# RNG65536/CUDA-volpath

Hardware: AMD Instinct MI355X
Metric: Msamples/sec (WxHxspp) + achieved HBM GB/s, Julia 256^3 @ 800x600 (higher is better)
Workload: dtype f32; 1 GPU; julia256_800x600_global_majorant; image=800x600, estimator=global_majorant, bound_brick=1, rng=philox2x32-7, parallelism=pixel-tiles x1

## Files before the change

cuda-volpath_amd/csrc/vp_context.cpp:

```cpp
#include "vp_state.h"

namespace vph __attribute__((visibility("hidden")))
{
State                      g_default;
static thread_local State* t_current = nullptr;
State& cur() { return t_current ? *t_current : g_default; }

int fail(int code, const char* fmt, ...)
{
    char    buf[512];
    va_list ap;
    va_start(ap, fmt);
    vsnprintf(buf, sizeof buf, fmt, ap);
    va_end(ap);
    G.err = buf;
    return code;
}
[[noreturn]] void die(const char* what)
{
    fprintf(stderr, "volpath_hip: %s: %s\n", what, G.err.c_str());
    exit(EXIT_FAILURE);
}
int ensure_device()
{
// ... 13 lines not shown
    G.num_cu = prop.multiProcessorCount;
    HIPCHK(hipStreamCreateWithFlags(&G.own_stream, hipStreamNonBlocking));
    if (!G.stream) G.stream = G.own_stream;
    HIPCHK(hipMalloc((void**)&G.d_queue, 2 * kTargets * kQueueWords * sizeof(unsigned)));
    HIPCHK(hipMalloc((void**)&G.d_counters, kCounterWords * sizeof(unsigned long long)));
    HIPCHK(hipMemset(G.d_counters, 0, kCounterWords * sizeof(unsigned long long)));
    HIPCHK(hipMalloc((void**)&G.d_cancel, 3 * sizeof(unsigned)));
    HIPCHK(hipMemset(G.d_cancel, 0, 3 * sizeof(unsigned)));
    G.S.sun_cos = 94.0f / sqrtf(94.0f * 94.0f + 0.45f * 0.45f);
    G.S.cam_z   = (float)(-1.0f / tan((double)54.43f * 0.00872664626));
    auto knob = [](const char* name, long lo, long hi, long& out) {
        const char* e = getenv(name);
        if (!e || !*e) return false;
        char* end = nullptr;
        long  v   = strtol(e, &end, 10);
        if (*end || v < lo || v > hi)
        {
            fprintf(stderr, "volpath_hip: ignoring %s=%s (allowed %ld..%ld)\n", name, e, lo, hi);
            return false;
        }
        out = v;
        return true;
    };
    long v;
    if (knob("VP_WAIT_LANES", 1, 64, v)) { G.wait_lanes = (unsigned)v; G.wait_lanes_set = true; }
    if (knob("VP_WAIT_ITERS", VP_STEPS_PER_PASS, 1 << 20, v)) G.wait_iters = (unsigned)v;
    if (knob("VP_SETUP_LANES", 1, 64, v)) G.setup_lanes = (unsigned)v;
    if (knob("VP_END_LANES", 1, 64, v)) G.end_lanes = (unsigned)v;
    if (knob("VP_LIGHT_WAIT_ITERS", VP_STEPS_PER_PASS, 1 << 20, v)) G.light_wait_iters = (unsigned)v;
    if (knob("VP_STAGE_MB", 1, 256 << 10, v)) G.max_stage_bytes = (size_t)v << 20;
    if (knob("VP_BLOCKS_PER_CU", 1, 8, v)) G.blocks_per_cu = (unsigned)v;
    {
        long kmax = 0;
        while ((VP_CHUNK >> (kmax + 1)) >= 1) kmax++;
        if (knob("VP_CHUNK_FRAMES_LOG2", 0, kmax, v)) G.chunk_fshift = (unsigned)v;
    }
    if (knob("VP_NO_LDS_BOUNDS", 0, 1, v)) G.use_lds_bounds = v == 0;
    if (knob("VP_NO_LDS_HELPER", 0, 1, v)) G.lds_helper = v == 0;
    if (knob("VP_NO_LDS_COMPACT", 0, 1, v)) G.use_lds_compact = v == 0;
    if (knob("VP_LDS_COMPACT_CHROMATIC", 0, 1, v)) G.lds_compact_chromatic = v != 0;
    if (knob("VP_LDS_PAIRS", 0, 1, v)) G.lds_pairs = v != 0;
    if (knob("VP_CELL_BRICKS", 0, 1, v)) G.cell_bricks = (int)v;
    if (knob("VP_NO_CRAWL_TABLE", 0, 1, v)) G.use_crawl_table = v == 0;
    if (knob("VP_NO_EMPTY_TABLE", 0, 1, v)) G.use_empty_table = v == 0;
    if (knob("VP_NO_SUN_CLIP", 0, 1, v)) G.use_sun_clip = v == 0;
    if (knob("VP_DENSE_PERCENT", 0, 101, v)) G.dense_fraction = (float)v / 100.0f;
    if (knob("VP_NO_OPACITY_LDS", 0, 1, v)) G.opacity_lds = v == 0;
    if (knob("VP_NO_OPACITY_CELLS", 0, 1, v)) G.use_opacity_cells = v == 0;
    if (knob("VP_NO_LIGHT_CONST", 0, 1, v)) G.use_light_const = v == 0;
    if (knob("VP_NO_CONST_ROWS", 0, 1, v)) G.use_const_rows = v == 0;
    if (knob("VP_NO_APPROACH", 0, 1, v)) G.use_approach = v == 0;
    if (knob("VP_NO_APPROACH_LOCAL", 0, 1, v)) G.use_approach_local = v == 0;
    if (knob("VP_NO_APPROACH_TABLE", 0, 1, v)) G.use_approach_table = v == 0;
    if (knob("VP_APPROACH_FRAMES_LOG2", 0, 6, v)) G.approach_fshift_max = (unsigned)v;
    if (knob("VP_APPROACH_STEPS", 0, 1 << 30, v)) G.approach_steps = (unsigned)v;
    if (knob("VP_NO_LIGHT", 0, 1, v)) G.use_light = v == 0;
    if (knob("VP_NO_LIGHT_OVERLAP", 0, 1, v)) G.light_overlap = v == 0;
    if (knob("VP_NO_LIGHT_LOCAL", 0, 1, v)) G.use_light_local = v == 0;
    if (knob("VP_DEBUG_ONLY_CLASS", 0, 1, v)) G.debug_only_class = (int)v;
    if (knob("VP_GENERAL_BLOCKS_PER_CU", 1, 8, v)) G.general_blocks_per_cu = (unsigned)v;
    if (knob("VP_LIGHT_BLOCKS_PER_CU", 1, 8, v)) G.light_blocks_per_cu = (unsigned)v;
    if (knob("VP_THR_TABLE", 2, 1 << 20, v)) G.thr_entries = (unsigned)v;
    if (knob("VP_LOOKAHEAD", 0, 4096, v)) G.la_max = (int)v;
    if (knob("VP_LOOKAHEAD_OVERLAP_FROM", 1, 4096, v)) G.la_overlap_from = (int)v;
    if (knob("VP_LOOKAHEAD_RAMP_FROM", 2, 4096, v)) G.la_ramp_from = (int)v;
    if (knob("VP_LOOKAHEAD_FLOOR", 1, 4096, v)) G.la_floor = (int)v;
    if (knob("VP_LOOKAHEAD_DIV", 1, 16, v)) G.la_div = (int)v;
    if (knob("VP_LOOKAHEAD_NO_SPECULATION", 0, 1, v)) G.la_speculate = v == 0;
    if (knob("VP_NO_LA_CANCEL", 0, 1, v)) G.la_cancel = v == 0;
    if (knob("VP_NO_PIPELINE", 0, 1, v)) G.pipeline = v == 0;
    if (knob("VP_NO_EXIT", 0, 1, v)) G.use_exit = v == 0;
    if (knob("VP_EXIT_LOCAL", 0, 1, v)) { G.exit_local = v != 0; G.exit_local_auto = false; }
    if (knob("VP_EXIT_K", 1, VP_EXIT_TRIP, v)) G.exit_k = (unsigned)v;
    G.dev_ready = true;
    return VP_OK;
}


hipError_t create_internal_stream(hipStream_t* st)
{
    int lo = 0, hi = 0;
    if (hipDeviceGetStreamPriorityRange(&lo, &hi) != hipSuccess) { (void)hipGetLastError(); lo = hi = 0; }
    return hipStreamCreateWithPriority(st, hipStreamNonBlocking, lo);
}

int free_volume()
{
    G.epoch++;
    (void)la_quiesce();

    if (G.d_cells) HIPCHK(hipFree(G.d_cells));
    if (G.d_bounds) HIPCHK(hipFree(G.d_bounds));
    if (G.d_opacity) HIPCHK(hipFree(G.d_opacity));
    if (G.d_opacity_cells) { if (G.opacity_cells_on_host) HIPCHK(hipHostFree(G.h_opacity_cells)); else HIPCHK(hipFree(G.d_opacity_cells)); }
    G.d_opacity_cells = nullptr; G.h_opacity_cells = nullptr; G.S.opacity_cells = nullptr; G.opacity_cells_on_host = false;
    if (G.d_bound_codes) HIPCHK(hipFree(G.d_bound_codes));
    G.d_bound_codes = nullptr; G.bound_codes_ok = false;
    if (G.d_danger) HIPCHK(hipFree(G.d_danger));
    G.d_danger = nullptr;
    if (G.d_sunclip) HIPCHK(hipFree(G.d_sunclip));
    G.d_sunclip = nullptr; G.sunclip_key.clear();
    if (G.d_exit) HIPCHK(hipFree(G.d_exit));
    G.d_exit = nullptr;
    G.d_cells = G.d_bounds = nullptr;
    G.d_opacity   = nullptr;
    G.S.cells_u8  = nullptr;
// ... 337 lines not shown
        fail(VP_E_NODEVICE, "vp_ctx_create: device %d not visible (%d devices)", device, n);
        return nullptr;
    }
    vp_ctx* c = new vp_ctx();
    c->st.device = device;
    State* prev = t_current;
    t_current   = &c->st;
    int rc      = ensure_device();
    std::string why = c->st.err;
    t_current   = prev;
    if (rc)
    {
        delete c;
        fail(rc, "vp_ctx_create(%d): %s", device, why.c_str());
        return nullptr;
    }
    return c;
}
int vp_ctx_set_current(vp_ctx* ctx)
{
    t_current = ctx ? &ctx->st : nullptr;
    if (G.dev_ready) HIPCHK(hipSetDevice(G.device));
    return VP_OK;
}
vp_ctx* vp_ctx_get_current(void) { return t_current ? reinterpret_cast<vp_ctx*>(t_current) : nullptr; }
int vp_ctx_device(void) { return G.device; }
int vp_ctx_destroy(vp_ctx* ctx)
{
    if (!ctx) return VP_OK;
    State* prev = t_current;
    t_current   = &ctx->st;
    State& D    = ctx->st;
    int rc = VP_OK;
    if (D.dev_ready)
    {
        (void)hipSetDevice(D.device);
        (void)hipStreamSynchronize(D.stream);
        (void)la_quiesce();
        rc = free_volume();
        free_envmap();
        for (auto& sl : D.la)
        {
            if (sl.done) (void)hipEventDestroy(sl.done);
            if (sl.stream) (void)hipStreamDestroy(sl.stream);
        }
        for (auto& ev : D.events) { (void)hipEventDestroy(ev.first); (void)hipEventDestroy(ev.second); }
        for (auto& ev : D.class_events) { (void)hipEventDestroy(ev.a); (void)hipEventDestroy(ev.b); }
        for (auto e : D.event_pool) (void)hipEventDestroy(e);
        (void)pipe_quiesce();
        for (hipStream_t st : D.pipe_stream) if (st) (void)hipStreamDestroy(st);
        for (hipEvent_t e : {D.pipe_done[0], D.pipe_done[1], D.pipe_free[0], D.pipe_free[1], D.pipe_gate[0], D.pipe_gate[1], D.pipe_fence_ev, D.last_end,
                             D.class_last_end[0], D.class_last_end[1], D.class_last_end[2]})
            if (e) (void)hipEventDestroy(e);
        D.d_crawl.release(); D.d_seg.release(); D.d_sub_cls.release(); D.d_tiles.release(); D.d_act.release(); D.d_act_scratch.release();
        for (void* q : {(void*)D.d_thr, (void*)D.d_sunclip, (void*)D.d_bound_codes, (void*)D.d_light_flag, (void*)D.d_tile_rows, (void*)D.d_tile_scratch})
            if (q) (void)hipFree(q);
        for (RenderTarget& t : D.target)
        {
            if (t.aux_stream) { (void)hipStreamSynchronize(t.aux_stream); (void)hipStreamDestroy(t.aux_stream); }
            t.stage.release();
            t.handover.release();
            for (hipEvent_t e : t.aux_ev) if (e) (void)hipEventDestroy(e);
        }
        if (D.d_queue) (void)hipFree(D.d_queue);
        if (D.d_counters) (void)hipFree(D.d_counters);
        if (D.ctrl_stream) (void)hipStreamDestroy(D.ctrl_stream);
        if (D.d_cancel) (void)hipFree(D.d_cancel);
        if (D.own_stream) (void)hipStreamDestroy(D.own_stream);
    }
    t_current = (prev == &ctx->st) ? nullptr : prev;
    delete ctx;
    if (G.dev_ready) (void)hipSetDevice(G.device);
    return rc;
}
int vp_accumulate(vp_float4* dst, const vp_float4* src, size_t n)
{
    int rc = ensure_device();
    if (rc) return rc;
    if (!dst || !src) return fail(VP_E_ARG, "vp_accumulate: null pointer");
    if (n) launch_accumulate((float4*)dst, (const float4*)src, n, G.stream);
    HIPCHK(hipGetLastError());
    return VP_OK;
}
int vp_tile_owner(unsigned tx, unsigned ty, int world)
{
    if (world < 1) return -1;
    return (int)((tx + vp::tile_row_shift(ty, (unsigned)world)) % (unsigned)world);
}
int vp_set_stream(void* s)
{
    int rc = ensure_device();
    if (rc) return rc;
    HIPCHK(hipStreamSynchronize(G.stream));
    if (la_quiesce()) return VP_E_NODEVICE;
    G.stream = s ? (hipStream_t)s : G.own_stream;
    return VP_OK;
}
void* vp_get_stream(void)
{
    if (ensure_device()) return nullptr;
    return (void*)G.stream;
}
int vp_synchronize(void)
{
    int rc = ensure_device();
    if (rc) return rc;
    HIPCHK(hipStreamSynchronize(G.stream));
// ... 12 lines not shown
    if (mode != VP_RNG_SAMPLERH && mode != VP_RNG_PHILOX && mode != VP_RNG_PHILOX7) return fail(VP_E_ARG, "unknown rng %d", mode);
    G.rng = mode; G.key0 = k0; G.key1 = k1;
    return VP_OK;
}
int vp_set_exit_flights(int mode)
{
    if (mode < 0 || mode > 2) return fail(VP_E_ARG, "exit flights: 0 off, 1 global-majorant estimator (default), 2 every estimator that has them");
    int rc = ensure_device();
    if (rc || (rc = pipe_quiesce())) return rc;
    G.use_exit = mode != 0; G.exit_local = mode == 2; G.exit_local_auto = false;
    if (G.use_exit && G.have_volume && !G.d_exit && G.d_danger)
    {
        if (la_quiesce()) return VP_E_NODEVICE;
        const size_t n = (size_t)G.S.nx * G.S.ny * G.S.nz;
        if (hipMalloc((void**)&G.d_exit, 3 * n) == hipSuccess)
        {
            launch_exit_table(G.d_danger, G.d_exit, G.S.nx, G.S.ny, G.S.nz, G.stream);
            HIPCHK(hipGetLastError());
        }
        else { (void)hipGetLastError(); G.d_exit = nullptr; }
    }
    return VP_OK;
}
int vp_set_tracking(int mode)
{
    if (int rc = pipe_quiesce()) return rc;
    if (mode != VP_TRACK_SPECTRAL && mode != VP_TRACK_SCALAR && mode != VP_TRACK_MULTI_CHANNEL)
        return fail(VP_E_ARG, "unknown tracking mode %d", mode);
    G.trk = mode;
    return VP_OK;
}
int vp_set_lookahead(int max_frames)
{
    if (max_frames < 0 || max_frames > 4096) return fail(VP_E_ARG, "look-ahead of %d frames out of range [0,4096]", max_frames);
    if (la_quiesce()) return VP_E_NODEVICE;
    G.la_max = max_frames; G.la_prev_n = 0;
    return VP_OK;
}
int vp_set_arithmetic(int mode)
{
    if (mode != VP_ARITH_EXACT && mode != VP_ARITH_FAST) return fail(VP_E_ARG, "unknown arithmetic mode %d", mode);
    if (mode == G.arith) return VP_OK;
    if (la_quiesce()) return VP_E_NODEVICE;
    G.arith = mode;
    return VP_OK;
}
int vp_set_subpixel(int s)
{
    const int shift = subpixel_shift_of(s);
    if (shift < 0) return fail(VP_E_ARG, "sub-pixel factor %d: 1, 2, 4 or 8", s);
    if (shift == G.sub_shift) return VP_OK;
    if (la_quiesce()) return VP_E_NODEVICE;
    G.sub_shift = shift;
    G.crawl_key.clear(); G.tiles_key.clear(); G.seg_key.clear();
    return VP_OK;
}
int vp_get_subpixel(void) { return 1 << G.sub_shift; }
int vp_subpixel_offset(unsigned x, unsigned y, int frame, int s, int* i, int* j)
{
    const int shift = subpixel_shift_of(s);
    if (shift < 0) return fail(VP_E_ARG, "sub-pixel factor %d: 1, 2, 4 or 8", s);
    if (x > 0xffffu || y > 0xffffu || frame < 0) return fail(VP_E_ARG, "vp_subpixel_offset: pixel (%u, %u) or frame %d out of range", x, y, frame);
    unsigned oi = 0, oj = 0;
    vp::subpixel_offset(x, y, (unsigned)frame, (unsigned)shift, oi, oj);
    if (i) *i = (int)oi;
    if (j) *j = (int)oj;
    return VP_OK;
}
int vp_set_envmap_sampling(int mode)
{
    if (int rc = pipe_quiesce()) return rc;
    if (mode != VP_ENV_PASSIVE && mode != VP_ENV_MIS) return fail(VP_E_ARG, "unknown environment sampling mode %d", mode);
    int rc = ensure_device();
    if (rc) return rc;
    G.env_mis = mode == VP_ENV_MIS;
    if (G.env_mis) return build_env_tables();
    return VP_OK;
}
int vp_get_env_tables(float* cdf_y, float* cdf_x, float* pdfnorm_alt)
{
    int rc = ensure_device();
    if (rc) return rc;
    if (!G.env_tables) return fail(VP_E_STATE, "no environment tables: vp_set_envmap_sampling(VP_ENV_MIS) and init_envmap first");
    HIPCHK(hipStreamSynchronize(G.stream));
    if (cdf_y) HIPCHK(hipMemcpy(cdf_y, G.d_env_cdf_y, (size_t)G.env_h * sizeof(float), hipMemcpyDeviceToHost));
    if (cdf_x) HIPCHK(hipMemcpy(cdf_x, G.d_env_cdf_x, (size_t)G.env_w * G.env_h * sizeof(float), hipMemcpyDeviceToHost));
    if (pdfnorm_alt) *pdfnorm_alt = G.S.env_pdfnorm_alt;
    return VP_OK;
}
int vp_init_volume(const void* h_volume, vp_extent ext, int format, const vp_float3* bmin, const vp_float3* bmax)
{
    if (!h_volume) return fail(VP_E_ARG, "vp_init_volume: null volume");
    if (format != VP_VOL_U8 && format != VP_VOL_F32 && format != VP_VOL_F16) return fail(VP_E_ARG, "vp_init_volume: unknown volume format %d", format);
    if (ext.width == 0 || ext.height == 0 || ext.depth == 0) return fail(VP_E_ARG, "empty volume extent");
    return do_init_volume(h_volume, ext, format, bmin, bmax);
}
int vp_get_volume_info(vp_volume_info* out)
{
    if (!out) return fail(VP_E_ARG, "vp_get_volume_info: null result");
    if (!G.have_volume) return fail(VP_E_STATE, "no volume");
    out->format = G.vol_format;
    out->nx = G.S.nx; out->ny = G.S.ny; out->nz = G.S.nz;
    out->cell_bytes  = G.quant ? 8 : (G.half() ? 16 : 32);
    out->cells_bytes = (uint64_t)G.cells_bytes;
    return VP_OK;
}
int vp_set_bound_brick(int brick)
// ... 162 lines not shown
    unsigned *dn = (unsigned*)D.get(c * 32), *dr = (unsigned*)D.get(c * 32);
    if (!dor || !db || !dn || !dr) return fail(VP_E_NOMEM, "vp_test_sun_start: no device memory");
    HIPCHK(hipMemcpy(dor, origin_xyz, c * 12, hipMemcpyHostToDevice));
    HIPCHK(hipMemcpy(db, box, 24, hipMemcpyHostToDevice));
    if (G.arith == VP_ARITH_FAST) launch_test_sun_start_fast(n, dor, sun_dir, db, dn, dr, G.stream);
    else launch_test_sun_start(n, dor, sun_dir, db, dn, dr, G.stream);
    HIPCHK(hipStreamSynchronize(G.stream));
    HIPCHK(hipMemcpy(out_new, dn, c * 32, hipMemcpyDeviceToHost));
    HIPCHK(hipMemcpy(out_ref, dr, c * 32, hipMemcpyDeviceToHost));
    return VP_OK;
}
int vp_test_hg(const float* g, const float* r0, const float* r1, const float* normal_xyz, const float* cos_query, float* dir_xyz, float* eval, int n)
{
    int rc = ensure_device();
    if (rc) return rc;
    if (n <= 0) return VP_OK;
    DevArrays D;
    const size_t b = (size_t)n * 4;
    float *dg = (float*)D.get(b), *d0 = (float*)D.get(b), *d1 = (float*)D.get(b), *dn = (float*)D.get(3 * b), *dc = (float*)D.get(b);
    float *dd = (float*)D.get(3 * b), *de = (float*)D.get(b);
    if (!dg || !d0 || !d1 || !dn || !dc || !dd || !de) return fail(VP_E_NOMEM, "vp_test_hg: no device memory");
    HIPCHK(hipMemcpy(dg, g, b, hipMemcpyHostToDevice));
    HIPCHK(hipMemcpy(d0, r0, b, hipMemcpyHostToDevice));
    HIPCHK(hipMemcpy(d1, r1, b, hipMemcpyHostToDevice));
    HIPCHK(hipMemcpy(dn, normal_xyz, 3 * b, hipMemcpyHostToDevice));
    HIPCHK(hipMemcpy(dc, cos_query, b, hipMemcpyHostToDevice));
    if (G.arith == VP_ARITH_FAST) launch_test_hg_fast(dg, d0, d1, dn, dc, dd, de, n, G.stream);
    else launch_test_hg(dg, d0, d1, dn, dc, dd, de, n, G.stream);
    HIPCHK(hipStreamSynchronize(G.stream));
    HIPCHK(hipMemcpy(dir_xyz, dd, 3 * b, hipMemcpyDeviceToHost));
    HIPCHK(hipMemcpy(eval, de, b, hipMemcpyDeviceToHost));
    return VP_OK;
}
int vp_test_intersect_box(const float* origin_xyz, const float* dir_xyz, int* hit, float* tnear, float* tfar, int n)
{
    if (!G.have_volume) return fail(VP_E_STATE, "no volume (the box comes from init_cuda)");
    int rc = ensure_device();
    if (rc) return rc;
    if (n <= 0) return VP_OK;
    DevArrays D;
    const size_t b = (size_t)n * 4;
    float *dor = (float*)D.get(3 * b), *ddi = (float*)D.get(3 * b), *dtn = (float*)D.get(b), *dtf = (float*)D.get(b);
    int*   dh  = (int*)D.get(b);
    if (!dor || !ddi || !dtn || !dtf || !dh) return fail(VP_E_NOMEM, "vp_test_intersect_box: no device memory");
    HIPCHK(hipMemcpy(dor, origin_xyz, 3 * b, hipMemcpyHostToDevice));
    HIPCHK(hipMemcpy(ddi, dir_xyz, 3 * b, hipMemcpyHostToDevice));
    launch_test_box(G.S, dor, ddi, dh, dtn, dtf, n, G.stream);
    HIPCHK(hipStreamSynchronize(G.stream));
    HIPCHK(hipMemcpy(hit, dh, b, hipMemcpyDeviceToHost));
    HIPCHK(hipMemcpy(tnear, dtn, b, hipMemcpyDeviceToHost));
    HIPCHK(hipMemcpy(tfar, dtf, b, hipMemcpyDeviceToHost));
    return VP_OK;
}
int vp_test_eval_envmap(const float* dir_xyz, float* rgb, int n)
{
    if (!G.have_env) return fail(VP_E_STATE, "no environment map");
    int rc = ensure_device();
    if (rc) return rc;
    if (n <= 0) return VP_OK;
    DevArrays D;
    const size_t b = (size_t)n * 12;
    float *dd = (float*)D.get(b), *dq = (float*)D.get(b);
    if (!dd || !dq) return fail(VP_E_NOMEM, "vp_test_eval_envmap: no device memory");
    HIPCHK(hipMemcpy(dd, dir_xyz, b, hipMemcpyHostToDevice));
    launch_test_env(G.S, dd, dq, n, G.stream);
    HIPCHK(hipStreamSynchronize(G.stream));
    HIPCHK(hipMemcpy(rgb, dq, b, hipMemcpyDeviceToHost));
    return VP_OK;
}

int vp_julia_voxelize(int n, unsigned char* host_out)
{
    int rc = ensure_device();
    if (rc) return rc;
    if (n < 1 || n > 1024 || !host_out) return fail(VP_E_ARG, "bad julia grid size %d", n);
    size_t total = (size_t)n * n * n;
    unsigned char* d = nullptr;
    HIPCHK(hipMalloc((void**)&d, total));
    launch_julia(d, n, G.stream);
    HIPCHK(hipGetLastError());
    HIPCHK(hipStreamSynchronize(G.stream));
    HIPCHK(hipMemcpy(host_out, d, total, hipMemcpyDeviceToHost));
    HIPCHK(hipFree(d));
    return VP_OK;
}

int vp_cloud_voxelize(int n, uint32_t seed, float* host_out)
{
    int rc = ensure_device();
    if (rc) return rc;
    if (n < 1 || n > 1024 || !host_out) return fail(VP_E_ARG, "bad cloud grid size %d", n);
    size_t total = (size_t)n * n * n;
    float* d = nullptr;
    HIPCHK(hipMalloc((void**)&d, total * sizeof(float)));
    launch_cloud(d, n, seed, G.stream);
    hipError_t e = hipGetLastError();
    if (e == hipSuccess) e = hipStreamSynchronize(G.stream);
    if (e == hipSuccess) e = hipMemcpy(host_out, d, total * sizeof(float), hipMemcpyDeviceToHost);
    (void)hipFree(d);
    if (e != hipSuccess) return fail(VP_E_NODEVICE, "vp_cloud_voxelize -> %s", hipGetErrorString(e));
    return VP_OK;
}

void* vp_malloc(size_t bytes)
{
    if (ensure_device()) return nullptr;
// ... 38 lines not shown
```

cuda-volpath_amd/csrc/vp_integrator.h:

```cpp
enum : int
{
    ST_DONE    = 0,
    ST_SETUP   = 1,
    ST_TRACK   = 2,
    ST_SHADOW  = 3,
    EV_SCATTER = 4,
    EV_NEE     = 5,
    EV_BG      = 6,
    EV_WRITE   = 7,
    EV_MIS     = 8,
    EV_HG      = 9
};

#ifndef VP_PAD_STEP
#define VP_PAD_STEP 0
#endif
#ifndef VP_PAD_FETCH
#define VP_PAD_FETCH 0
#endif
#ifndef VP_PAD_EOF
#define VP_PAD_EOF 0
#endif
#ifndef VP_PAD_SETUP
#define VP_PAD_SETUP 0
// ... 90 lines not shown
    {
        const float reduction   = (1.0f - s) + s * (1.0f - P.g);
        const float cur_density = reduction * P.density;
        const float d_max       = fmaxf(0.0001f, (float)b * VP_U8_SCALE);
        sigma_t_prime           = max_sig * cur_density * d_max;
    }
    else
    {
        const float cur_density = (1.0f - s) * P.density + s * P.density * (1.0f - P.g);
        sigma_t_prime           = max_sig * cur_density;
    }
    const float inv_sigma_t = rcp_(sigma_t_prime);
    if (!(null_collision_in_empty_space(1.0f, sigma_t_prime, inv_sigma_t) == 1.0f)) atomicAnd(flag, 0u);
}

#ifndef VP_LOCAL_MIN_WAVES
#define VP_LOCAL_MIN_WAVES 6
#endif
constexpr int render_min_waves(int est, bool count, int ldsb, bool ach, bool mis, int trk, bool light, bool cancel)
{
    if (VP_MIN_WAVES > 1) return VP_MIN_WAVES;
    if (light) return count ? 5 : (est != EST_GLOBAL ? VP_LIGHT_LOCAL_MIN_WAVES : VP_LIGHT_MIN_WAVES);
    if (mis || ldsb == 1) return 1;
    if (count) return 4;
    if (est == EST_GLOBAL && trk == 0) return VP_GLOBAL_MIN_WAVES;
    if (trk) return 4;
    return (ach && !cancel) ? VP_LOCAL_MIN_WAVES : 5;
}
#define VP_RENDER_K_HAS_LAYERS 1
template <int EST, class RNG, bool QUANT, bool COUNT, int LDSB, bool ACH, bool MIS, int TRK, bool LIGHT = false, bool CANCEL = false, bool HALF = false, bool LYR = false>
__global__ __launch_bounds__(LDSB == 1 ? VP_BLOCK_LDS : VP_BLOCK, render_min_waves(EST, COUNT, LDSB, ACH, MIS, TRK, LIGHT, CANCEL))
void render_k(SceneDev S, LaunchDev L)
{
    __shared__ unsigned short lds_bounds[LDSB == 1 ? VP_LDS_BOUND_ENTRIES : 1];
    __shared__ unsigned lds_codes[LDSB == 2 ? VP_LDS_BOUND_ENTRIES / 16 : 1];
    if (LDSB == 2)
    {
        const uint4* src = reinterpret_cast<const uint4*>(L.bound_codes);
        uint4*       dst = reinterpret_cast<uint4*>(lds_codes);
        const int    n16 = (S.bnx * S.bny * S.bnz + 63) / 64;
        for (int w = threadIdx.x; w < n16; w += VP_BLOCK) dst[w] = src[w];
        __syncthreads();
    }
    if (LDSB == 1)
    {
        const uint4* src = reinterpret_cast<const uint4*>(S.bounds_u8);
        uint4*       dst = reinterpret_cast<uint4*>(lds_bounds);
        const int    n16 = (S.bnx * S.bny * S.bnz * 2 + 15) / 16;
        for (int w = threadIdx.x; w < n16; w += VP_BLOCK_LDS) dst[w] = src[w];
        __syncthreads();
    }
    constexpr unsigned KARG_L_   = ((sizeof(SceneDev) + alignof(LaunchDev) - 1) / alignof(LaunchDev)) * alignof(LaunchDev);
    constexpr unsigned KARG_WDS_ = (KARG_L_ + sizeof(LaunchDev) + 3) / 4;
    constexpr bool LOCAL = EST != EST_GLOBAL;
    constexpr bool TAB   = TRK == 0 && LDSB != 1 && !LIGHT && !MIS;
#ifdef VP_EXP_BOX_PARALLEL
    constexpr bool SUNROW = false;
#else
    constexpr bool SUNROW = TAB && EST != EST_BOUNDED;
#endif
    __shared__ __attribute__((aligned(16))) unsigned kargs_lds_[KARG_WDS_ + (SUNROW ? SR_WORDS : 0)];
    {
        const unsigned* src = (const unsigned*)__builtin_amdgcn_kernarg_segment_ptr();
        for (unsigned w = threadIdx.x; w < KARG_WDS_; w += (LDSB == 1 ? VP_BLOCK_LDS : VP_BLOCK)) kargs_lds_[w] = src[w];
    }
    __shared__ __attribute__((aligned(16))) float coll_tab_[TAB ? VP_COLL_ROWS : 1][CR_WORDS];
    if (TAB && threadIdx.x < VP_COLL_ROWS)
        coll_row_fill(coll_tab_[threadIdx.x], (int)threadIdx.x, L.P.g, L.P.density, max3(f3{L.P.sigma_t[0], L.P.sigma_t[1], L.P.sigma_t[2]}), LOCAL);
    if (SUNROW && threadIdx.x == VP_COLL_ROWS)
        sun_row_fill(reinterpret_cast<float*>(kargs_lds_ + KARG_WDS_), f3{S.sun_dir[0], S.sun_dir[1], S.sun_dir[2]});
    __syncthreads();
    auto coll_row = [&](int n) __attribute__((always_inline)) -> const float* {
        return TAB ? coll_tab_[n < 0 ? 0 : (n > VP_COLL_ROWS - 1 ? VP_COLL_ROWS - 1 : n)] : nullptr;
    };
    constexpr bool EARLY = RNG::kShadowSubstream && !MIS && !LIGHT;
    constexpr bool APPR = EST == EST_GLOBAL && TRK == 0 && !LIGHT && !MIS;
    constexpr bool APPR_L = EST == EST_DECOMP && TRK == 0 && !LIGHT && !MIS;
    constexpr bool EXITC = TRK == 0 && !MIS && !LIGHT && EST != EST_BOUNDED && (QUANT || EST == EST_GLOBAL);
    constexpr bool PARK = !MIS;
    constexpr bool DEFER = EARLY && TRK == 0;
    constexpr bool LAYERS = LYR;
    static_assert(!LYR || (TRK == 0 && !MIS && !COUNT && !CANCEL), "layers instances: spectral tracking, passive environment, no counters, no look-ahead");
    const ParamDev& P = L.P;
    const f3    sig_t     = f3{P.sigma_t[0], P.sigma_t[1], P.sigma_t[2]};
    const f3    sig_s     = sig_t * f3{P.albedo[0], P.albedo[1], P.albedo[2]};
    const float max_sig   = max3(sig_t);
    const float min_sig   = min3(sig_t);
    const float density   = P.density;

    int      st = ST_DONE;
    bool     exhausted = false;
    constexpr bool COLD = LDSB != 1 && !LIGHT;
    constexpr int  CS_  = COLD ? VP_BLOCK : 1;
    constexpr int NCOLD = 14 + (DEFER ? (ACH ? 1 : 3) : 0);
    static_assert(!COLD || (LOCAL ? VP_LOCAL_MIN_WAVES : VP_GLOBAL_MIN_WAVES) * (NCOLD * VP_BLOCK * 4 + KARG_WDS_ * 4 + VP_COLL_ROWS * CR_WORDS * 4 + (SUNROW ? SR_WORDS * 4 : 0) + (LDSB == 2 ? VP_LDS_BOUND_ENTRIES / 4 : 0)) <= VP_LDS_BYTES_PER_CU,
                  "cold per-path state: more workgroups per CU than the LDS holds -- lower VP_*_MIN_WAVES for this ARCH");
    __shared__ float cold_[COLD ? NCOLD : 1][CS_];
    float* const cold_p = &cold_[0][COLD ? threadIdx.x : 0];
    ColdF3<COLD, CS_>       rad(cold_p), pd(cold_p + 3 * CS_);
    ColdVal<float, COLD>    ph(cold_p + 6 * CS_), phase_g(cold_p + 7 * CS_);
    ColdVal<unsigned, COLD> item(cold_p + 8 * CS_);
    ColdVal<unsigned, COLD> px(cold_p + 9 * CS_), py(cold_p + 10 * CS_);
    ColdVal<int, COLD>      frame(cold_p + 11 * CS_);
    ColdVal<int, COLD>      nsc(cold_p + 12 * CS_);
    ColdVal<unsigned, COLD> rng_saved(cold_p + 13 * CS_);
    constexpr unsigned LIGHT_NONE = 0xffffffffu;
    ColdVal<float, COLD>    lw_x(cold_p + 6 * CS_), lw_y(cold_p + (DEFER && !ACH ? 14 : 6) * CS_), lw_z(cold_p + (DEFER && !ACH ? 15 : 6) * CS_);
    ColdVal<unsigned, COLD> light_bits(cold_p + (DEFER ? NCOLD - 1 : 6) * CS_);
    if (COLD) { rad = f3{0.0f, 0.0f, 0.0f}; pd = f3{0.0f, 0.0f, 0.0f}; ph = 0.0f; phase_g = 0.0f; item = 0u; px = 0u; py = 0u; frame = 0; nsc = 0; rng_saved = 0u; }
    if (DEFER) { lw_x = 0.0f; if (!ACH) { lw_y = 0.0f; lw_z = 0.0f; } light_bits = LIGHT_NONE; }
    RNG      rng;
    f3       ro = {}, rd = {};
    f3       inv_rd = {};
    f3       thr = {};
    int      seg = 0;
    float    dist = 0, t_end = 0;
    float    t_far = 0, distc = 0, inv_sigma = 0, inv_sigma_t = 0, sigma_t_prime = 0, sigma_c = 0;
    float    cur_density = 0, d_max = 0;
    f3       nee_a = {};
    int      terms = 0;
    f3       nee_c = {}, nee_t = {}, seg_o = {};
    int      nee_stage = 0;
    float    sh_inv_sigma = 0, sh_density = 0;
    float    sig_base = density;
    int      chan = 0;
    float    t_empty = 0.0f;
    float    t_clip = 1e30f;
    bool     ex_clear = false;
    unsigned long long c_load = 0, c_xtest = 0, c_xout = 0, c_xok = 0;
    unsigned zrun = 0;

    unsigned long long c_den = 0, c_bnd = 0, c_opa = 0, c_env = 0, c_sca = 0, c_smp = 0;
    unsigned long long d_iter = 0, d_act = 0, d_outer = 0, d_shadow = 0;
    constexpr bool PROF = COUNT && VP_PROFILE_BLOCKS;
    unsigned long long t_slow = 0, t_fast = 0, t_mark = PROF ? __builtin_amdgcn_s_memtime() : 0ull;
    enum { B_SETUP, B_HALF, B_LOOK, B_EXIT, B_SCATTER, B_NEE, B_HG, B_BG, B_WRITE, B_REFILL, B_GSETUP, B_FETCH, B_ZERO, B_ZERO_SH, B_EXITT, B_NBLK };
    unsigned long long bw[B_NBLK] = {}, bl[B_NBLK] = {};
    unsigned long long hist[3][8] = {};
    unsigned long long ctrl_w = 0, ctrl_l = 0;
    auto tally = [&](int b, bool on) __attribute__((always_inline)) {
        if (PROF)
        {
            unsigned long long m = __ballot(on);
            if (m)
            {
                bw[b] += 1; bl[b] += (unsigned)__popcll(m);
                const int h = b == B_SCATTER ? 0 : b == B_EXIT ? 1 : b == B_SETUP ? 2 : -1;
                if (h >= 0) hist[h][((unsigned)__popcll(m) - 1u) >> 3] += 1;
            }
        }
    };

    const unsigned lane = threadIdx.x & 63u;
    unsigned chunk_s = 0, chunk_n = 0;
    unsigned chunk_q = 0, chunk_f0 = 0;
    bool     queue_empty = false;
    unsigned q_cur   = __builtin_amdgcn_s_getreg((4 - 1) << 11 | 20) & (VP_NQUEUES - 1);
    unsigned q_tried = 0;
    unsigned end_skipped = 0;
    unsigned visits = 0;

    for (;;)
    {
        if (PROF && lane == 0) d_outer++;
        {
#ifdef VP_EXP_FLAT_KARGS
        const char* kargs_ = (const char*)__builtin_amdgcn_kernarg_segment_ptr();
        asm volatile("" : "+s"(kargs_));
#else
        unsigned ko_ = 0;
        asm volatile("" : "+v"(ko_));
        const char* kargs_ = reinterpret_cast<const char*>(kargs_lds_) + ko_;
#endif
        const SceneDev&  S = *reinterpret_cast<const SceneDev*>(kargs_);
        const LaunchDev& L = *reinterpret_cast<const LaunchDev*>(kargs_ + KARG_L_);
        const ParamDev&  P = L.P;
        const f3 sun_dir   = f3{S.sun_dir[0], S.sun_dir[1], S.sun_dir[2]};
        const f3 sun_power = f3{S.sun_power[0], S.sun_power[1], S.sun_power[2]};
        auto start_shadow = [&](f3 end, float inv_s, float den, unsigned stage) __attribute__((always_inline)) {
            f3    sd;
            float len, tn, tf;
            bool  hitv;
            if (SUNROW && stage == 0u)
            {
#ifdef VP_EXP_FLAT_KARGS
                const float* const srow = reinterpret_cast<const float*>(kargs_lds_ + KARG_WDS_);
#else
                const float* const srow = reinterpret_cast<const float*>(kargs_ + KARG_WDS_ * 4u);
#endif
                hitv = sun_start(srow, ro, S.bmin, S.bmax, sd, len, tn, tf);
            }
            else
            {
                const f3    dv = end - ro;
                const float d2 = dot(dv, dv);
                len = sqrt_(d2);
#ifdef VP_ARITH_FAST
                sd = dv * rsqrt_(d2);
#else
                sd = dv * rcp_(len);
#endif
                hitv = intersect_box(ro, sd, S, tn, tf);
            }
            if (!hitv)
            {
                nee_a = f3{1.0f, 1.0f, 1.0f};
                st    = EV_NEE;
            }
            else
            {
                if (tn < 0.0f) tn = 0.0f;
                t_end       = fminf(tf, len);
                dist        = tn;
                terms       = 0;
                rd          = sd;
                inv_sigma   = inv_s;
                cur_density = den;
                st          = ST_SHADOW;
                rng_saved = rng.enter_shadow(2u * (unsigned)(int)nsc + stage);
                if (COUNT) t_clip = 1e30f;
                if (RNG::kShadowSubstream && stage == 0u && L.sun_clip)
                {
                    f3    pl = to_local(S, ro);
                    int   ci, cj, ck;
                    float w_;
                    axis_linear(pl.x, S.nx, ci, w_);
                    axis_linear(pl.y, S.ny, cj, w_);
                    axis_linear(pl.z, S.nz, ck, w_);
                    const unsigned n = L.sun_clip[(size_t)((unsigned)ci + __umul24((unsigned)S.nx, (unsigned)cj + __umul24((unsigned)S.ny, (unsigned)ck)))];
                    if (n != 0xffffu)
                    {
                        const float tc = (float)n * L.clip_ds;
                        if (COUNT && !L.count_clips) t_clip = tc;
                        else t_end = fminf(t_end, tc);
                    }
                }
            }
        };
        auto segment_medium = [&]() __attribute__((always_inline)) {
            if (LOCAL && TAB) cur_density = coll_row(nsc - 5)[CR_DENS];
            else if (LOCAL)
// ... 210 lines not shown
                const f3 pl = to_local(S, st == ST_TRACK ? ro + rd * dist : ro);
                int   ci, cj, ck;
                float w_;
                axis_linear(pl.x, S.nx, ci, w_);
                axis_linear(pl.y, S.ny, cj, w_);
                axis_linear(pl.z, S.nz, ck, w_);
                const float ex = rd.x * (S.linv[0] * (float)S.nx), ey = rd.y * (S.linv[1] * (float)S.ny), ez = rd.z * (S.linv[2] * (float)S.nz);
                const float ax = __builtin_fabsf(ex), ay = __builtin_fabsf(ey), az = __builtin_fabsf(ez);
                const unsigned A   = (ax >= ay && ax >= az) ? 0u : (ay >= az ? 1u : 2u);
                const unsigned cls = A == 0u ? ((ex > 0.0f ? 1u : 0u) | (ey > 0.0f ? 2u : 0u) | (ez > 0.0f ? 4u : 0u))
                                   : A == 1u ? ((ey > 0.0f ? 1u : 0u) | (ex > 0.0f ? 2u : 0u) | (ez > 0.0f ? 4u : 0u))
                                             : ((ez > 0.0f ? 1u : 0u) | (ex > 0.0f ? 2u : 0u) | (ey > 0.0f ? 4u : 0u));
                const size_t   ncell = (size_t)S.nx * (size_t)S.ny * (size_t)S.nz;
                const unsigned bits  = L.exit_oct[(size_t)A * ncell + (size_t)((unsigned)ci + __umul24((unsigned)S.nx, (unsigned)cj + __umul24((unsigned)S.ny, (unsigned)ck)))];
                bool clear = (bits >> cls) & 1u;
                bool unit = true;
                if (clear)
                {
                    const f3 t3 = ACH ? f3{thr.x, thr.x, thr.x} : thr;
                    if (LOCAL)
                    {
                        for (unsigned q = 0; q < L.exit_nbytes; q++)
                        {
                            const float dm  = fmaxf(0.0001f, (float)((L.exit_bytes >> (8u * q)) & 0xffu) * VP_U8_SCALE);
                            const float stp = max_sig * cur_density * dm;
                            unit = unit && null_collision_is_identity(t3, stp, rcp_(stp));
                        }
                    }
                    else
                        unit = null_collision_is_identity(t3, sigma_t_prime, inv_sigma_t);
                }
                if (COUNT && clear && unit) c_xok++;
                if (clear && unit && !(COUNT && !L.count_clips)) st = EV_BG;
                else
                {
                    if (COUNT && clear && unit) ex_clear = true;
                    terms = (clear && unit) ? -(1 << 30) : (unit ? L.exit_start : L.exit_start - 4 * VP_EXIT_TRIP);
                }
            }
        }
        {
            const unsigned long long wantm = __ballot(st == EV_BG || st == EV_WRITE || (st == ST_DONE && !exhausted) || (EST == EST_GLOBAL && st == ST_SETUP));
            const bool fast_any = __ballot(st == ST_TRACK || st == ST_SHADOW || (LOCAL && st == ST_SETUP)) != 0ull;
            end_skipped++;
            if (wantm == 0ull || (!LIGHT && fast_any && (unsigned)__popcll(wantm) < L.end_lanes && end_skipped < 4u)) goto ends_done;
            end_skipped = 0u;
        }
#pragma unroll 1
        for (int rep = 0; rep < 4; rep++)
        {
            vp_pad<VP_PAD_END>();
            bool fresh = false;
            bool trans = false;
            tally(B_BG, st == EV_BG);
            if (st == EV_BG)
            {
                if (!MIS || nsc == 0)
                {
                    if (LAYERS) trans = nsc == 0;
                    f3 bg;
                    if (LAYERS && trans) bg = f3{1.0f, 1.0f, 1.0f};
                    else if (nsc == 0 && dot(rd, sun_dir) > S.sun_cos) bg = f3{S.sun_orig[0], S.sun_orig[1], S.sun_orig[2]};
                    else { bg = eval_envmap(S, rd); if (COUNT) c_env++; }
                    if (LIGHT && !LOCAL)
                    {
                        const unsigned n = (unsigned)seg, last = L.thr_n - 1u;
                        float t = L.thr_table[n < last ? n : last];
                        for (unsigned k = last; k < n; k++) t = null_collision_in_empty_space(t, sigma_t_prime, inv_sigma_t);
                        thr = f3{t, t, t};
                    }
                    rad = rad + bg * (ACH ? f3{thr.x, thr.x, thr.x} : thr);
                }
                st = EV_WRITE;
            }
            tally(B_WRITE, st == EV_WRITE);
            if (st == EV_WRITE)
            {
                f3     r    = rad * ((LAYERS && trans) ? 1.0f : P.brightness);
#ifdef VP_ARITH_FAST
                r = f3{r.x < __builtin_inff() ? r.x : 0.0f, r.y < __builtin_inff() ? r.y : 0.0f, r.z < __builtin_inff() ? r.z : 0.0f};
#endif
                float  heat = (EST == EST_DECOMP) ? (float)nsc : (float)((double)(EST == EST_BOUNDED ? seg : nsc) * 0.001);
                if (LAYERS && !LIGHT && trans) heat = -heat;
                float4 v    = make_float4(fmaxf(r.x, 0.0f), fmaxf(r.y, 0.0f), fmaxf(r.z, 0.0f), heat);
                if (TRK == 2)
                    v = make_float4(chan == 0 ? v.x * 3.0f : 0.0f, chan == 1 ? v.y * 3.0f : 0.0f, chan == 2 ? v.z * 3.0f : 0.0f, heat);
                if (L.stage) L.stage[item] = v;
                else
                {
                    size_t idx = (size_t)px + (size_t)py * P.width;
                    float4 a   = L.out[idx];
                    L.out[idx] = make_float4(a.x + v.x, a.y + v.y, a.z + v.z, a.w + v.w);
                }
                st = ST_DONE;
            }
            {
                bool               need = (st == ST_DONE) && !exhausted;
                unsigned long long m    = __ballot(need);
                tally(B_REFILL, need);
                if (m)
                {
                    while (chunk_s >= chunk_n && !queue_empty)
                    {
                        const unsigned q0 = L.q_start[q_cur], len = L.q_start[q_cur + 1] - q0;
                        static_assert((VP_CHUNK & (VP_CHUNK - 1)) == 0 && VP_CHUNK >= 64, "VP_CHUNK: a power of two, at least a wave");
                        const unsigned sh = L.chunk_fshift, ppc = (unsigned)VP_CHUNK >> sh, fblocks = (unsigned)L.nframes >> sh;
                        const unsigned cpf = (len + ppc - 1u) / ppc;
                        unsigned c = 0xffffffffu;
                        if (len)
                        {
                            if (lane == 0 && !(L.cancel && __hip_atomic_load(L.cancel, __ATOMIC_RELAXED, __HIP_MEMORY_SCOPE_AGENT) >= L.batch_id)) c = atomicAdd(L.queue + q_cur * VP_QUEUE_STRIDE, 1u);
                            c = __builtin_amdgcn_readfirstlane(c);
                        }
                        if (c < cpf * fblocks)
                        {
                            const unsigned pos = c / fblocks, fb = c - pos * fblocks, off = pos * ppc;
                            chunk_q  = q0 + off;
                            chunk_f0 = fb << sh;
                            chunk_n  = (len - off < ppc ? len - off : ppc) << sh;
                            chunk_s  = 0;
                        }
                        else
                        {
                            q_cur = (q_cur + 1) & (VP_NQUEUES - 1);
                            if (++q_tried >= VP_NQUEUES) queue_empty = true;
                        }
                    }
                    unsigned cnt   = (unsigned)__popcll(m);
                    unsigned avail = chunk_n - chunk_s;
                    unsigned take  = cnt < avail ? cnt : avail;
                    unsigned rank  = lane_rank(m);
                    if (need)
                    {
                        if (rank >= take) { if (queue_empty) exhausted = true;  }
                        else
                        {
                            const unsigned sn  = chunk_s + rank, sh = L.chunk_fshift;
                            const unsigned rem = chunk_q + (sn >> sh);
                            const unsigned fl  = chunk_f0 + (sn & ((1u << sh) - 1u));
                            item = fl * L.stage_stride + L.slot_base + rem;
                            unsigned pix = L.pixels[rem];
                            px    = pix & 0xffffu;
                            py    = pix >> 16;
                            frame = L.frame0 + (int)fl;
                            if (px < P.width && py < P.height)
                            {
                                auto table_index = [&]() -> size_t
                                {
                                    if (!COUNT && L.sub_shift)
                                    {
                                        unsigned si, sj;
                                        subpixel_offset(px, py, (unsigned)frame, L.sub_shift, si, sj);
                                        return (size_t)((px << L.sub_shift) + si) + (size_t)((py << L.sub_shift) + sj) * (P.width << L.sub_shift);
                                    }
                                    return (size_t)px + (size_t)py * P.width;
                                };
                                if (!COUNT && L.sub_shift)
                                {
                                    unsigned si, sj;
                                    subpixel_offset(px, py, (unsigned)frame, L.sub_shift, si, sj);
                                    const unsigned fx = (px << L.sub_shift) + si, fy = (py << L.sub_shift) + sj;
                                    rng.init(fx, fy, (unsigned)frame, L.key0, L.key1);
                                    camera_ray(S, P.width << L.sub_shift, P.height << L.sub_shift, fx, fy, ro, rd);
                                }
                                else
                                {
                                    rng.init(px, py, (unsigned)frame, L.key0, L.key1);
                                    camera_ray(S, P.width, P.height, px, py, ro, rd);
                                }
                                if (TRK == 2)
                                {
                                    chan     = (int)fminf((1.0f - rng.next_a()) * 3.0f, 2.9999998f);
                                    sig_base = density * (chan == 0 ? P.sigma_t[0] : chan == 1 ? P.sigma_t[1] : P.sigma_t[2]);
                                }
                                if (LOCAL) inv_rd = f3{1.0f / rd.x, 1.0f / rd.y, 1.0f / rd.z};
                                thr = f3{1.0f, 1.0f, 1.0f};
                                rad = f3{0.0f, 0.0f, 0.0f};
                                nsc = 0;
                                seg = 0;
                                if (EXITC) terms = L.exit_start;
                                if (COUNT) ex_clear = false;
                                if (!LIGHT) t_empty = L.crawl ? L.crawl[2 * table_index() + 1].x : 0.0f;
                                if (LOCAL) dist = -1.0f;
                                if (APPR && L.approach)
                                {
                                    const float4 a = L.stage[item];
                                    dist  = a.x;
                                    rng.load(f2u(a.y), f2u(a.z));
                                    fresh = true;
                                    if (L.approach == 2u)
                                    {
                                        const unsigned n = f2u(a.w), last = L.thr_n - 1u;
                                        float t = L.thr_table[n < last ? n : last];
                                        if (n > last)
                                        {
                                            const float s0  = hyperion_s(0 - 5);
                                            const float stp = max_sig * ((1.0f - s0) * density + s0 * density * (1.0f - P.g));
                                            const float inv = rcp_(stp);
                                            for (unsigned k = last; k < n; k++) t = null_collision_in_empty_space(t, stp, inv);
                                        }
                                        thr = f3{t, t, t};
                                    }
                                }
                                if (LOCAL && L.crawl)
                                {
                                    float4   c = L.crawl[2 * table_index()];
                                    unsigned k = f2u(c.w);
                                    ro = f3{c.x, c.y, c.z};
                                    if (!(APPR_L && L.approach)) rng.skip(k >> 16);
                                    if (EST == EST_BOUNDED) seg = (int)(k & 0xffffu);
                                    if (COUNT) c_bnd += k & 0xffffu;
                                    if (APPR_L && L.approach)
                                    {
                                        const float4 a  = L.stage[item];
                                        const uint2  ax = L.approach_aux[item];
                                        const f3     ra = f3{a.x, a.y, a.z};
                                        t_empty = t_empty - dot(ra - ro, rd) - 1e-4f;
                                        ro      = ra;
                                        dist    = a.w;
                                        rng.load(ax.x, ax.y);
                                    }
                                }
                                st  = ST_SETUP;
                                segment_medium();
                                if (COUNT) c_smp++;
                            }
                        }
                    }
                    chunk_s += take;
                }
            }
            if (EST == EST_GLOBAL) tally(B_GSETUP, st == ST_SETUP);
            if (EST == EST_GLOBAL && st == ST_SETUP)
            {
                float t_near, tf;
                bool  hit = intersect_box(ro, rd, S, t_near, tf);
                if (!hit) st = EV_BG;
                else
                {
                    if (t_near < 0.0f) t_near = 0.0f;
                    t_far         = tf;
                    t_end         = tf;
                    dist          = (APPR && fresh) ? dist : t_near;
                    float s       = hyperion_s(nsc - 5);
                    if (!TAB) phase_g = (1.0f - s) * P.g;
                    if (TAB)
                    {
                        const float* const row = coll_row(nsc - 5);
                        cur_density   = row[CR_DENS];
                        sigma_t_prime = row[CR_STP];
                    }
                    else if (TRK)
                    {
                        sigma_t_prime = (1.0f - s) * sig_base + s * sig_base * (1.0f - P.g);
                        cur_density   = sigma_t_prime;
                    }
                    else
                    {
                        cur_density   = (1.0f - s) * density + s * density * (1.0f - P.g);
                        sigma_t_prime = max_sig * cur_density;
                    }
                    inv_sigma     = TAB ? coll_row(nsc - 5)[CR_INV] : rcp_(sigma_t_prime);
                    inv_sigma_t   = inv_sigma;
                    st            = ST_TRACK;
                }
            }
            if (__ballot((st == ST_DONE && !exhausted) || st == EV_BG || st == EV_WRITE) == 0ull) break;
        }
ends_done:
        if (CANCEL && L.cancel && (visits++ & 7u) == 0u)
        {
            unsigned w = 0;
            if (lane == 0) w = __hip_atomic_load(L.cancel, __ATOMIC_RELAXED, __HIP_MEMORY_SCOPE_AGENT);
            if ((unsigned)__builtin_amdgcn_readfirstlane((int)w) >= L.batch_id) { st = ST_DONE; exhausted = true; queue_empty = true; }
        }
        if (__ballot(st != ST_DONE || !exhausted) == 0ull) break;
        }
        if (PROF) { unsigned long long t = __builtin_amdgcn_s_memtime(); if (lane == 0) t_slow += t - t_mark; t_mark = t; }

        auto segment_setup = [&]() __attribute__((always_inline)) {
            if (LOCAL) tally(B_SETUP, st == ST_SETUP);
            if (LOCAL && st == ST_SETUP)
            {
                vp_pad<VP_PAD_SETUP>();
                float t_near, tf;
                bool  hit = intersect_box_inv(ro, inv_rd, S, t_near, tf);
                t_near    = fmaxf(t_near, 0.0f);
                t_far     = fminf(tf, 0.05f);
                float bx, by;
// ... 636 lines not shown
```

cuda-volpath_amd/csrc/vp_kernels.h:

```cpp
#pragma once
#include <hip/hip_runtime.h>

#include "vp_device.h"

#define VP_BLOCK 256
#ifndef VP_BLOCK_LDS
#define VP_BLOCK_LDS 512
#endif
#ifndef VP_MIN_WAVES
#define VP_MIN_WAVES 1
#endif
#define VP_LDS_BYTES_PER_CU (160 * 1024)
#define VP_LDS_BOUND_ENTRIES 32768
#ifndef VP_CHUNK
#define VP_CHUNK 128
#endif
#define VP_NQUEUES 8
#define VP_QUEUE_STRIDE 16
#ifndef VP_WAIT_LANES
#define VP_WAIT_LANES 28
#endif
#ifndef VP_WAIT_ITERS
#define VP_WAIT_ITERS 16
#endif
// ... 21 lines not shown
#ifndef VP_STEPS_PER_PASS
#define VP_STEPS_PER_PASS 4
#endif
#define VP_EXIT_TRIP 64

namespace vp
{
__host__ __device__ inline unsigned tile_row_shift(unsigned ty, unsigned world) { return ((ty * 0x9E3779B1u) >> 15) % world; }
constexpr int EST_GLOBAL = 0, EST_DECOMP = 1, EST_BOUNDED = 2;
constexpr int RNG_SAMPLERH = 0, RNG_PHILOX = 1, RNG_PHILOX7 = 2;

struct LaunchDev
{
    ParamDev P;
    int      frame0, nframes;
    unsigned nslots;
    unsigned total_items;
    const unsigned* pixels;
    unsigned stage_stride;
    unsigned slot_base;
    float4*  out;
    float4*  stage;
    const float4* crawl;
    unsigned* queue;
    unsigned chunk_fshift;
    unsigned q_start[VP_NQUEUES + 1];
    unsigned long long* counters;
    unsigned key0, key1;
    unsigned wait_lanes, wait_iters;
    unsigned end_lanes;
    unsigned setup_lanes;
    const unsigned short* sun_clip;
    float    clip_ds;
    unsigned count_clips;
    const float* thr_table;
    unsigned thr_n;
    uint2*   approach_aux;
    unsigned approach;
    unsigned approach_fshift;
    unsigned approach_steps;
    const unsigned char* exit_oct;
    int      exit_start;
    unsigned exit_nbytes;
    unsigned exit_bytes;
    unsigned* cancel;
    unsigned  batch_id;
    unsigned      const_from;
    const float4* stage_const;
    const unsigned* bound_codes;
    unsigned        bound_pal[2];
    const float4* seg_table;
    unsigned sub_shift;
    unsigned layers;
};

[[noreturn]] void kernel_not_built();
constexpr int CENSUS_RENDER = 0, CENSUS_LAYERS = 1, CENSUS_APPROACH = 2;
void census_record(int unit, int kind, unsigned index);
size_t census_size(int kind);
void census_read(int unit, int kind, unsigned* launches, unsigned char* built, size_t count, bool reset);
void census_built(int kind, unsigned char* built, size_t count);
void census_built_fast(int kind, unsigned char* built, size_t count);
void launch_render(const SceneDev& S, const LaunchDev& L, int est, int rng, bool quant, bool half, bool count, int lds_form, bool mis, int trk,
                   int blocks, hipStream_t st);
void launch_render_fast(const SceneDev& S, const LaunchDev& L, int est, int rng, bool quant, bool half, bool count, int lds_form, bool mis, int trk,
                        int blocks, hipStream_t st);
void launch_render_light(const SceneDev& S, const LaunchDev& L, int est, int rng, bool quant, bool count, int blocks, hipStream_t st);
void launch_miss_fill(const SceneDev& S, const LaunchDev& L, bool local_estimator, hipStream_t st);
void launch_approach(const SceneDev& S, const LaunchDev& L, int est, int rng, bool quant, hipStream_t st);
void launch_approach_fast(const SceneDev& S, const LaunchDev& L, int est, int rng, bool quant, hipStream_t st);
unsigned segment_table_records(void);
void launch_segment_table(const SceneDev& S, unsigned width, unsigned height, const float4* crawl, const unsigned* pixels, unsigned nslots, float4* seg,
                          hipStream_t st);
void launch_thr_table(const ParamDev& P, float* table, unsigned count, hipStream_t st);
void launch_bound_bytes(const unsigned char* bounds, size_t nbricks, unsigned* mask, hipStream_t st);
void launch_light_identity(const ParamDev& P, bool local, const unsigned* mask, unsigned* flag, hipStream_t st);
void launch_light_identity_fast(const ParamDev& P, bool local, const unsigned* mask, unsigned* flag, hipStream_t st);
inline unsigned pixel_list_blocks(unsigned ntiles) { return (unsigned)(((size_t)ntiles * 64 + 1023) / 1024); }
void launch_pixel_lists(unsigned width, unsigned height, unsigned rank, unsigned world, unsigned ntiles, const unsigned* d_row_start,
                        const float4* table, const unsigned char* cls, unsigned* d_block_counts, unsigned* d_totals, unsigned* d_out, hipStream_t st);
void launch_subpixel_classes(const float4* fine, unsigned width, unsigned height, unsigned shift, unsigned char* cls, hipStream_t st);
void launch_env_tables(const float4* env, int w, int h, float* lum, float* row_sum, float* cdf_x, float* cdf_y, float* pdfnorm_alt,
                       hipStream_t st);
void launch_crawl_table(const SceneDev& S, bool quant, unsigned width, unsigned height, bool control_draw, const unsigned char* danger, float4* table,
                        hipStream_t st);
void launch_danger(const SceneDev& S, bool quant, bool half, unsigned char* out, unsigned long long* marked, hipStream_t st);
float sun_clip_step(const SceneDev& S);
void launch_sun_clip(const SceneDev& S, const unsigned char* danger, float ds, unsigned short* out, hipStream_t st);
void launch_empty_table(const SceneDev& S, unsigned width, unsigned height, const unsigned char* danger, float4* table, hipStream_t st);
void launch_exit_table(const unsigned char* danger, unsigned char* planes, int nx, int ny, int nz, hipStream_t st);
void launch_reduce(const LaunchDev& L, hipStream_t st);
void launch_reduce_layers(const LaunchDev& L, float4* trans, unsigned light_from, unsigned light_to, hipStream_t st);
struct PixelStatsDev { double sum_y, sum_y2; unsigned n, flags; };
struct StatsDev
{
    PixelStatsDev* stats;
    unsigned adaptive;
    unsigned min_frames;
    double   tol, fl;
};
void launch_reduce_stats(const LaunchDev& L, const StatsDev& T, hipStream_t st);
inline unsigned compact_blocks(unsigned n) { return (n + 1023u) / 1024u; }
void launch_compact_active(const unsigned* src, const unsigned n[3], unsigned width, const PixelStatsDev* stats, unsigned* d_block_counts,
                           unsigned* d_totals, unsigned* d_out, hipStream_t st);
void launch_scale_by_count(float4* dst, const float4* src, const PixelStatsDev* stats, int size, float s, hipStream_t st);
void launch_stats_rel_error(float* dst, const PixelStatsDev* stats, int size, float floor_y, hipStream_t st);
size_t denoise_lds_bytes(int R, int F);
void launch_denoise(float4* dst, const float4* src, const PixelStatsDev* stats, const float4* guide, const PixelStatsDev* gstats, int W, int H, int R,
                    int F, float k2, int form, hipStream_t st);
void launch_pack_u8(const unsigned char* vol, uint2* cells, int nx, int ny, int nz, bool bricks, hipStream_t st);
void launch_pack_f32(const float* vol, float* cells, int nx, int ny, int nz, bool bricks, hipStream_t st);
void launch_pack_f16(const unsigned short* vol, uint4* cells, int nx, int ny, int nz, bool bricks, hipStream_t st);
void launch_opacity(const SceneDev& S, bool quant, bool half, bool lds, const float dir[3], float* out, hipStream_t st);
void launch_build_bounds(const void* d_vol, bool quant, bool half, void* d_out, void* d_tmp_a, void* d_tmp_b, int nx, int ny, int nz, int radius, int brick,
                         hipStream_t st);
void launch_julia(unsigned char* grid, int n, hipStream_t st);
void launch_cloud(float* grid, int n, unsigned seed, hipStream_t st);
void launch_scale(float4* dst, const float4* src, int size, float s, hipStream_t st);
void launch_composite(float4* dst, const float4* fg, const float4* trans, const float4* plate, float r, float g, float b, int size, float s, hipStream_t st);
void launch_gamma(float4* dst, const float4* src, int size, float s, float inv_gamma, hipStream_t st);
void launch_accumulate(float4* dst, const float4* src, size_t n, hipStream_t st);
void launch_test_hg(const float* g, const float* r0, const float* r1, const float* nrm, const float* cosq, float* dir, float* ev, int n, hipStream_t st);
void launch_test_box(const SceneDev& S, const float* o, const float* d, int* hit, float* tn, float* tf, int n, hipStream_t st);
void launch_test_env(const SceneDev& S, const float* d, float* out, int n, hipStream_t st);
void launch_test_math(int which, const float* in, float* out, int n, hipStream_t st);
void launch_test_roots(int which, unsigned lo, unsigned hi, unsigned long long* mismatches, unsigned* first_bad, hipStream_t st);
void launch_test_hg_fast(const float* g, const float* r0, const float* r1, const float* nrm, const float* cosq, float* dir, float* ev, int n, hipStream_t st);
void launch_test_math_fast(int which, const float* in, float* out, int n, hipStream_t st);
void launch_test_log_forms(int which, unsigned lo, unsigned hi, unsigned long long* mismatches, unsigned* first_bad, hipStream_t st);
void launch_test_log_forms_fast(int which, unsigned lo, unsigned hi, unsigned long long* mismatches, unsigned* first_bad, hipStream_t st);
void launch_test_approach_walk(int kind, int n, const float* par, const unsigned* scr, const unsigned* words, unsigned* out_new, unsigned* out_ref, hipStream_t st);
void launch_test_approach_walk_fast(int kind, int n, const float* par, const unsigned* scr, const unsigned* words, unsigned* out_new, unsigned* out_ref,
                                    hipStream_t st);
void launch_test_sun_start(int n, const float* origin, const float* sun_dir, const float* box, unsigned* out_new, unsigned* out_ref, hipStream_t st);
void launch_test_sun_start_fast(int n, const float* origin, const float* sun_dir, const float* box, unsigned* out_new, unsigned* out_ref, hipStream_t st);
void launch_test_rng(int mode, unsigned x, unsigned y, unsigned f, unsigned k0, unsigned k1, int n, float* out, hipStream_t st);
void launch_test_density(const SceneDev& S, bool quant, bool half, const float* pos, float* out, int n, hipStream_t st);
}
```

cuda-volpath_amd/csrc/vp_kernels.hip:

```cpp
#include <hip/hip_runtime.h>

#include <atomic>
#include <cmath>
#include <cstdint>
#include <cstdio>
#include <cstdlib>
#include <utility>

#include "vp_device.h"
#include "vp_kernels.h"

namespace vp
{
#include "vp_integrator.h"

__global__ void thr_table_k(ParamDev P, float* table, unsigned count)
{
    if (threadIdx.x || blockIdx.x) return;
    const float max_sig       = max3(f3{P.sigma_t[0], P.sigma_t[1], P.sigma_t[2]});
    const float s             = hyperion_s(0 - 5);
    const float cur_density   = (1.0f - s) * P.density + s * P.density * (1.0f - P.g);
    const float sigma_t_prime = max_sig * cur_density;
    const float inv_sigma_t   = 1.0f / sigma_t_prime;
    float t = 1.0f;
// ... 563 lines not shown
    const unsigned k = t / L.nslots, slot = t - k * L.nslots;
    const ParamDev& P = L.P;
    const unsigned pix = L.pixels[slot], px = pix & 0xffffu, py = pix >> 16;
    const unsigned h = wang_hash(((px << 16) | py) ^ 0x9E3779B9u);
    unsigned fl = (k - ((unsigned)L.frame0 + h)) & (n2 - 1u);
    if (fl >= (unsigned)L.nframes) return;
    unsigned i, j;
    subpixel_offset(px, py, (unsigned)L.frame0 + fl, m, i, j);
    f3 ro, rd;
    camera_ray(S, P.width << m, P.height << m, (px << m) + i, (py << m) + j, ro, rd);
    bool env_lookup = false;
    const float4 v = unscattered_sample(S, P, rd, env_lookup, L.layers);
    if (L.stage)
        for (; fl < (unsigned)L.nframes; fl += n2) L.stage[(size_t)fl * L.stage_stride + L.slot_base + slot] = v;
    else
    {
        size_t idx = (size_t)px + (size_t)py * P.width;
        float4 a   = L.out[idx];
        L.out[idx] = make_float4(a.x + v.x, a.y + v.y, a.z + v.z, a.w + v.w);
    }
}

__global__ __launch_bounds__(256) void approach_segments_k(SceneDev S, unsigned width, unsigned height, const float4* crawl, const unsigned* pixels,
                                                           unsigned nslots, float4* seg)
{
    const unsigned slot = blockIdx.x * blockDim.x + threadIdx.x;
    if (slot >= nslots) return;
    float4* out = seg + (size_t)slot * (2 * VP_SEG_CAP);
    const unsigned pix = pixels[slot], px = pix & 0xffffu, py = pix >> 16;
    if (px >= width || py >= height) { out[0] = make_float4(0.0f, 0.0f, u2f(0x100u), 0.0f); out[VP_SEG_CAP] = make_float4(0.0f, 0.0f, 0.0f, 0.0f); return; }
    f3 ro, rd;
    camera_ray(S, width, height, px, py, ro, rd);
    const f3     inv_rd = f3{1.0f / rd.x, 1.0f / rd.y, 1.0f / rd.z};
    const size_t idx    = (size_t)px + (size_t)py * width;
    const float4 c      = crawl[2 * idx];
    float        t_empty = crawl[2 * idx + 1].x;
    ro                  = f3{c.x, c.y, c.z};
    for (unsigned n = 0; n < VP_SEG_CAP; n++)
    {
        float t_near, tf;
        const bool hit = intersect_box_inv(ro, inv_rd, S, t_near, tf);
        t_near         = fmaxf(t_near, 0.0f);
        const float t_far = fminf(tf, 0.05f);
        const f3  pl = to_local(S, ro + rd * t_near);
        const int bi = axis_point(pl.x, S.nx) >> S.brick_shift, bj = axis_point(pl.y, S.ny) >> S.brick_shift, bk = axis_point(pl.z, S.nz) >> S.brick_shift;
        const unsigned v = reinterpret_cast<const unsigned short*>(S.bounds_u8)[(size_t)((unsigned)bi + (unsigned)S.bnx * ((unsigned)bj + (unsigned)S.bny * (unsigned)bk))];
        const bool stop = !hit || (v >> 8) != 0u || n == VP_SEG_CAP - 1u;
        out[n]              = make_float4(t_near, t_far, u2f((v & 0xffu) | (stop ? 0x100u : 0u)), t_empty);
        out[VP_SEG_CAP + n] = make_float4(ro.x, ro.y, ro.z, 0.0f);
        if (stop) break;
        ro      = ro + rd * t_far;
        t_empty -= t_far;
    }
}

__device__ __forceinline__ size_t pack_index(int nx, int ny, int i, int j, int k, int bricks)
{
    if (!bricks) return (size_t)i + (size_t)nx * ((size_t)j + (size_t)ny * k);
    const size_t nbx = ((size_t)nx + 3) >> 2, nby = ((size_t)ny + 3) >> 2;
    return ((((size_t)i >> 2) + nbx * (((size_t)j >> 2) + nby * ((size_t)k >> 2))) << 6) | (size_t)(((k & 3) << 4) | ((j & 3) << 2) | (i & 3));
}
__global__ void pack_cells_u8_k(const unsigned char* vol, uint2* cells, int nx, int ny, int nz, int bricks)
{
    size_t n   = (size_t)nx * ny * nz;
    size_t idx = (size_t)blockIdx.x * blockDim.x + threadIdx.x;
    if (idx >= n) return;
    int i = (int)(idx % nx), j = (int)((idx / nx) % ny), k = (int)(idx / ((size_t)nx * ny));
    int i1 = i + 1 < nx ? i + 1 : nx - 1, j1 = j + 1 < ny ? j + 1 : ny - 1, k1 = k + 1 < nz ? k + 1 : nz - 1;
    auto at = [&](int a, int b, int c) -> unsigned { return vol[(size_t)a + (size_t)nx * ((size_t)b + (size_t)ny * c)]; };
    uint2 c;
    c.x = at(i, j, k) | (at(i1, j, k) << 8) | (at(i, j1, k) << 16) | (at(i1, j1, k) << 24);
    c.y = at(i, j, k1) | (at(i1, j, k1) << 8) | (at(i, j1, k1) << 16) | (at(i1, j1, k1) << 24);
    cells[pack_index(nx, ny, i, j, k, bricks)] = c;
}
__global__ void pack_cells_f32_k(const float* vol, float* cells, int nx, int ny, int nz, int bricks)
{
    size_t n   = (size_t)nx * ny * nz;
    size_t idx = (size_t)blockIdx.x * blockDim.x + threadIdx.x;
    if (idx >= n) return;
    int i = (int)(idx % nx), j = (int)((idx / nx) % ny), k = (int)(idx / ((size_t)nx * ny));
    int i1 = i + 1 < nx ? i + 1 : nx - 1, j1 = j + 1 < ny ? j + 1 : ny - 1, k1 = k + 1 < nz ? k + 1 : nz - 1;
    auto at = [&](int a, int b, int c) -> float { return vol[(size_t)a + (size_t)nx * ((size_t)b + (size_t)ny * c)]; };
    float4* q = reinterpret_cast<float4*>(cells) + pack_index(nx, ny, i, j, k, bricks) * 2;
    q[0] = make_float4(at(i, j, k), at(i1, j, k), at(i, j1, k), at(i1, j1, k));
    q[1] = make_float4(at(i, j, k1), at(i1, j, k1), at(i, j1, k1), at(i1, j1, k1));
}
__global__ void pack_f16_k(const unsigned short* vol, uint4* cells, int nx, int ny, int nz, int bricks)
{
    size_t n   = (size_t)nx * ny * nz;
    size_t idx = (size_t)blockIdx.x * blockDim.x + threadIdx.x;
    if (idx >= n) return;
    int i = (int)(idx % nx), j = (int)((idx / nx) % ny), k = (int)(idx / ((size_t)nx * ny));
    int i1 = i + 1 < nx ? i + 1 : nx - 1, j1 = j + 1 < ny ? j + 1 : ny - 1, k1 = k + 1 < nz ? k + 1 : nz - 1;
    auto at = [&](int a, int b, int c) -> unsigned { return vol[(size_t)a + (size_t)nx * ((size_t)b + (size_t)ny * c)]; };
    cells[pack_index(nx, ny, i, j, k, bricks)] = make_uint4(at(i, j, k) | (at(i1, j, k) << 16), at(i, j1, k) | (at(i1, j1, k) << 16),
                                                            at(i, j, k1) | (at(i1, j, k1) << 16), at(i, j1, k1) | (at(i1, j1, k1) << 16));
}

struct PairU8
{
    typedef unsigned char  T;
    typedef unsigned short P;
    static __device__ __forceinline__ P make(T mx, T mn) { return (P)((unsigned)mx | ((unsigned)mn << 8)); }
    static __device__ __forceinline__ T mx(P p) { return (T)(p & 0xffu); }
    static __device__ __forceinline__ T mn(P p) { return (T)(p >> 8); }
};
// ... 348 lines not shown
    if (c && index < census_size(kind)) c[index].fetch_add(1u, std::memory_order_relaxed);
}
void census_read(int unit, int kind, unsigned* launches, unsigned char* built, size_t count, bool reset)
{
    std::atomic<uint32_t>* c = census_counters(unit, kind);
    if (!c) return;
    if (count > census_size(kind)) count = census_size(kind);
    if (built) { if (unit) census_built_fast(kind, built, count); else census_built(kind, built, count); }
    for (size_t i = 0; i < count; i++)
    {
        const uint32_t n = reset ? c[i].exchange(0u, std::memory_order_relaxed) : c[i].load(std::memory_order_relaxed);
        if (launches) launches[i] = n;
    }
}
void census_built(int kind, unsigned char* built, size_t count) { dispatch_census_built(kind, built, count); }
void launch_render(const SceneDev& S, const LaunchDev& L, int est, int rng, bool quant, bool half, bool count, int lds_form, bool mis, int trk,
                   int blocks, hipStream_t st)
{
    dispatch_render(S, L, est, rng, quant, half, count, lds_form, mis, trk, blocks, st);
}
void launch_render_light(const SceneDev& S, const LaunchDev& L, int est, int rng, bool quant, bool count, int blocks, hipStream_t st)
{
    dispatch_light(S, L, est, rng, quant, count, blocks, st);
}
void launch_approach(const SceneDev& S, const LaunchDev& L, int est, int rng, bool quant, hipStream_t st) { dispatch_approach(S, L, est, rng, quant, st); }
void launch_bound_bytes(const unsigned char* bounds, size_t nbricks, unsigned* mask, hipStream_t st)
{
    unsigned blocks = (unsigned)std::fmin((double)((nbricks + 255) / 256), 1024.0);
    hipLaunchKernelGGL(bound_bytes_k, dim3(blocks ? blocks : 1), dim3(256), 0, st, reinterpret_cast<const unsigned short*>(bounds), nbricks, mask);
}
void launch_light_identity(const ParamDev& P, bool local, const unsigned* mask, unsigned* flag, hipStream_t st)
{
    hipLaunchKernelGGL(light_identity_k, dim3(1), dim3(256), 0, st, P, local ? 1 : 0, mask, flag);
}
void launch_thr_table(const ParamDev& P, float* table, unsigned count, hipStream_t st)
{
    hipLaunchKernelGGL(thr_table_k, dim3(1), dim3(64), 0, st, P, table, count);
}
void launch_miss_fill(const SceneDev& S, const LaunchDev& L, bool local_estimator, hipStream_t st)
{
    if (L.sub_shift)
    {
        hipLaunchKernelGGL(subpixel_fill_k, dim3(((L.nslots << (2u * L.sub_shift)) + 255) / 256), dim3(256), 0, st, S, L);
        return;
    }
    hipLaunchKernelGGL(miss_fill_k, dim3((L.nslots + 255) / 256), dim3(256), 0, st, S, L, local_estimator ? 1 : 0);
}
unsigned segment_table_records(void) { return 2u * VP_SEG_CAP; }
void launch_segment_table(const SceneDev& S, unsigned width, unsigned height, const float4* crawl, const unsigned* pixels, unsigned nslots, float4* seg,
                          hipStream_t st)
{
    hipLaunchKernelGGL(approach_segments_k, dim3((nslots + 255u) / 256u), dim3(256), 0, st, S, width, height, crawl, pixels, nslots, seg);
}
void launch_pixel_lists(unsigned width, unsigned height, unsigned rank, unsigned world, unsigned ntiles, const unsigned* d_row_start,
                        const float4* table, const unsigned char* cls, unsigned* d_block_counts, unsigned* d_totals, unsigned* d_out, hipStream_t st)
{
    PixListDev D;
    D.cls = cls;
    D.width = width; D.height = height; D.rank = rank; D.world = world;
    D.tiles_x = (width + 7) / 8; D.tiles_y = (height + 7) / 8; D.ntiles = ntiles; D.row_start = d_row_start; D.table = table;
    const unsigned nblocks = pixel_list_blocks(ntiles);
    if (!nblocks) return;
    hipLaunchKernelGGL(pixlist_count_k, dim3(nblocks), dim3(VP_PIXLIST_BLOCK), 0, st, D, d_block_counts);
    hipLaunchKernelGGL(pixlist_scan_k, dim3(1), dim3(VP_PIXLIST_BLOCK), 0, st, d_block_counts, nblocks, d_totals);
    hipLaunchKernelGGL(pixlist_write_k, dim3(nblocks), dim3(VP_PIXLIST_BLOCK), 0, st, D, (const unsigned*)d_block_counts, (const unsigned*)d_totals, d_out);
}

__global__ void env_lum_k(const float4* env, float* lum, int w, int h)
{
    int i = blockIdx.x * blockDim.x + threadIdx.x;
    if (i >= w * h) return;
    int    y   = i / w;
    float  phi = kPi * ((float)y + 0.5f) / (float)h;
    float  sp, cp;
    sincosf_(phi, sp, cp);
    float4 t = env[i];
    lum[i]   = luminance(f3{t.x, t.y, t.z}) * sp;
}
__global__ void env_row_cdf_k(const float* lum, float* cdf_x, float* row_sum, int w, int h)
{
    int y = blockIdx.x * blockDim.x + threadIdx.x;
    if (y >= h) return;
    const float* f   = lum + (size_t)y * w;
    float*       cdf = cdf_x + (size_t)y * w;
    float        sum = 0.0f;
    for (int i = 0; i < w; i++) sum += f[i];
    float norm = 1.0f / sum;
    float I    = 0.0f;
    for (int i = 0; i < w; i++) { I += f[i] * norm; cdf[i] = I; }
    cdf[w - 1] = 1.0f;
    row_sum[y] = sum;
}
__global__ void env_col_cdf_k(const float* lum, const float* row_sum, float* cdf_y, float* pdfnorm_alt, int w, int h)
{
    if (blockIdx.x || threadIdx.x) return;
    float lumsum = 0.0f;
    for (size_t i = 0, n = (size_t)w * h; i < n; i++) lumsum += lum[i];
    *pdfnorm_alt = (float)w * (float)h * k1TwoPiPi / lumsum;
    float sum = 0.0f;
    for (int i = 0; i < h; i++) sum += row_sum[i];
    float norm = 1.0f / sum;
    float I    = 0.0f;
    for (int i = 0; i < h; i++) { I += row_sum[i] * norm; cdf_y[i] = I; }
    cdf_y[h - 1] = 1.0f;
}
void launch_env_tables(const float4* env, int w, int h, float* lum, float* row_sum, float* cdf_x, float* cdf_y, float* pdfnorm_alt,
// ... 148 lines not shown
void launch_cloud(float* grid, int n, unsigned seed, hipStream_t st)
{
    size_t total = (size_t)n * n * n;
    hipLaunchKernelGGL(cloud_k, dim3((unsigned)((total + 255) / 256)), dim3(256), 0, st, grid, n, seed);
}
void launch_composite(float4* dst, const float4* fg, const float4* trans, const float4* plate, float r, float g, float b, int size, float s, hipStream_t st)
{
    hipLaunchKernelGGL(composite_k, dim3((size + 255) / 256), dim3(256), 0, st, dst, fg, trans, plate, r, g, b, size, s);
}
void launch_scale(float4* dst, const float4* src, int size, float s, hipStream_t st)
{
    hipLaunchKernelGGL(scale_k, dim3((size + 255) / 256), dim3(256), 0, st, dst, src, size, s);
}
void launch_gamma(float4* dst, const float4* src, int size, float s, float inv_gamma, hipStream_t st)
{
    hipLaunchKernelGGL(gamma_k, dim3((size + 255) / 256), dim3(256), 0, st, dst, src, size, s, inv_gamma);
}
void launch_accumulate(float4* dst, const float4* src, size_t n, hipStream_t st)
{
    hipLaunchKernelGGL(accumulate_k, dim3((unsigned)((n + 255) / 256)), dim3(256), 0, st, dst, src, n);
}
void launch_test_hg(const float* g, const float* r0, const float* r1, const float* nrm, const float* cosq, float* dir, float* ev, int n, hipStream_t st)
{
    hipLaunchKernelGGL(test_hg_k, dim3((n + 255) / 256), dim3(256), 0, st, g, r0, r1, nrm, cosq, dir, ev, n);
}
void launch_test_box(const SceneDev& S, const float* o, const float* d, int* hit, float* tn, float* tf, int n, hipStream_t st)
{
    hipLaunchKernelGGL(test_box_k, dim3((n + 255) / 256), dim3(256), 0, st, S, o, d, hit, tn, tf, n);
}
void launch_test_env(const SceneDev& S, const float* d, float* out, int n, hipStream_t st)
{
    hipLaunchKernelGGL(test_env_k, dim3((n + 255) / 256), dim3(256), 0, st, S, d, out, n);
}
void launch_test_math(int which, const float* in, float* out, int n, hipStream_t st)
{
    hipLaunchKernelGGL(test_math_k, dim3((n + 255) / 256), dim3(256), 0, st, which, in, out, n);
}
void launch_test_roots(int which, unsigned lo, unsigned hi, unsigned long long* mismatches, unsigned* first_bad, hipStream_t st)
{
    hipLaunchKernelGGL(test_roots_k, dim3(2048), dim3(256), 0, st, which, lo, hi, mismatches, first_bad);
}
void launch_test_log_forms(int which, unsigned lo, unsigned hi, unsigned long long* mismatches, unsigned* first_bad, hipStream_t st)
{
    hipLaunchKernelGGL(test_log_forms_k, dim3(2048), dim3(256), 0, st, which, lo, hi, mismatches, first_bad);
}
void launch_test_approach_walk(int kind, int n, const float* par, const unsigned* scr, const unsigned* words, unsigned* out_new, unsigned* out_ref, hipStream_t st)
{
    hipLaunchKernelGGL(test_approach_walk_k, dim3((n + 63) / 64), dim3(64), 0, st, kind, n, par, scr, words, out_new, out_ref);
}
void launch_test_sun_start(int n, const float* origin, const float* sun_dir, const float* box, unsigned* out_new, unsigned* out_ref, hipStream_t st)
{
    hipLaunchKernelGGL(test_sun_start_k, dim3((n + 255) / 256), dim3(256), 0, st, n, origin, sun_dir[0], sun_dir[1], sun_dir[2], box, out_new, out_ref);
}
void launch_test_rng(int mode, unsigned x, unsigned y, unsigned f, unsigned k0, unsigned k1, int n, float* out, hipStream_t st)
{
    if (mode == RNG_PHILOX) hipLaunchKernelGGL(test_rng_k<RngPhilox>, dim3(1), dim3(64), 0, st, x, y, f, k0, k1, n, out);
    else if (mode == RNG_PHILOX7) hipLaunchKernelGGL(test_rng_k<RngPhilox7>, dim3(1), dim3(64), 0, st, x, y, f, k0, k1, n, out);
    else hipLaunchKernelGGL(test_rng_k<RngSamplerH>, dim3(1), dim3(64), 0, st, x, y, f, k0, k1, n, out);
}
void launch_test_density(const SceneDev& S, bool quant, bool half, const float* pos, float* out, int n, hipStream_t st)
{
    if (quant) hipLaunchKernelGGL(test_density_k<true>, dim3((n + 255) / 256), dim3(256), 0, st, S, pos, out, n);
    else if (half) hipLaunchKernelGGL((test_density_k<false, true>), dim3((n + 255) / 256), dim3(256), 0, st, S, pos, out, n);
    else hipLaunchKernelGGL(test_density_k<false>, dim3((n + 255) / 256), dim3(256), 0, st, S, pos, out, n);
}
}
```

cuda-volpath_amd/csrc/vp_kernels_fast.hip:

```cpp
#define VP_ARITH_FAST 1

#include <hip/hip_runtime.h>

#include <cstdio>
#include <cstdlib>
#include <utility>

#include "vp_device.h"
#include "vp_kernels.h"

namespace vp
{
namespace fast
{
#include "vp_integrator.h"
#include "vp_test_kernels.h"

#include "vp_dispatch.h"
}

void launch_render_fast(const SceneDev& S, const LaunchDev& L, int est, int rng, bool quant, bool half, bool count, int lds_form, bool mis, int trk,
                        int blocks, hipStream_t st)
{
    fast::dispatch_render(S, L, est, rng, quant, half, count, lds_form, mis, trk, blocks, st);
}

void launch_light_identity_fast(const ParamDev& P, bool local, const unsigned* mask, unsigned* flag, hipStream_t st)
{
    hipLaunchKernelGGL(fast::light_identity_k, dim3(1), dim3(256), 0, st, P, local ? 1 : 0, mask, flag);
}

void launch_approach_fast(const SceneDev& S, const LaunchDev& L, int est, int rng, bool quant, hipStream_t st) { fast::dispatch_approach(S, L, est, rng, quant, st); }
void census_built_fast(int kind, unsigned char* built, size_t count) { fast::dispatch_census_built(kind, built, count); }

void launch_test_hg_fast(const float* g, const float* r0, const float* r1, const float* nrm, const float* cosq, float* dir, float* ev, int n, hipStream_t st)
{
    hipLaunchKernelGGL(fast::test_hg_k, dim3((n + 255) / 256), dim3(256), 0, st, g, r0, r1, nrm, cosq, dir, ev, n);
}
void launch_test_math_fast(int which, const float* in, float* out, int n, hipStream_t st)
{
    hipLaunchKernelGGL(fast::test_math_k, dim3((n + 255) / 256), dim3(256), 0, st, which, in, out, n);
}
void launch_test_log_forms_fast(int which, unsigned lo, unsigned hi, unsigned long long* mismatches, unsigned* first_bad, hipStream_t st)
{
    hipLaunchKernelGGL(fast::test_log_forms_k, dim3(2048), dim3(256), 0, st, which, lo, hi, mismatches, first_bad);
}
void launch_test_approach_walk_fast(int kind, int n, const float* par, const unsigned* scr, const unsigned* words, unsigned* out_new, unsigned* out_ref,
                                    hipStream_t st)
{
    hipLaunchKernelGGL(fast::test_approach_walk_k, dim3((n + 63) / 64), dim3(64), 0, st, kind, n, par, scr, words, out_new, out_ref);
}
void launch_test_sun_start_fast(int n, const float* origin, const float* sun_dir, const float* box, unsigned* out_new, unsigned* out_ref, hipStream_t st)
{
    hipLaunchKernelGGL(fast::test_sun_start_k, dim3((n + 255) / 256), dim3(256), 0, st, n, origin, sun_dir[0], sun_dir[1], sun_dir[2], box, out_new, out_ref);
}
}
```

cuda-volpath_amd/csrc/vp_render.cpp:

```cpp
#include "vp_state.h"

namespace vph __attribute__((visibility("hidden")))
{
static float span_ms(hipEvent_t a, hipEvent_t b, hipEvent_t& end)
{
    float ms = 0.0f, since = 0.0f;
    if (hipEventElapsedTime(&ms, a, b) != hipSuccess) { (void)hipGetLastError(); return 0.0f; }
    if (end && hipEventElapsedTime(&since, end, b) == hipSuccess)
    {
        if (since <= 0.0f) return 0.0f;
        ms = std::min(ms, since);
    }
    else (void)hipGetLastError();
    end = b;
    return std::max(ms, 0.0f);
}
static void fold_span(hipEvent_t a, hipEvent_t b, hipEvent_t& end, double& sum)
{
    hipEvent_t e = end;
    if (hipEventQuery(b) == hipSuccess) sum += span_ms(a, b, e);
    else (void)hipGetLastError();
    put_event(a);
    if (e == b) { put_event(end); end = b; }
    else put_event(b);
// ... 114 lines not shown
}
static int pipe_await_launch(int ps, hipStream_t st)
{
    HIPCHK(hipEventRecord(G.pipe_done[ps], st));
    HIPCHK(hipStreamWaitEvent(G.stream, G.pipe_done[ps], 0));
    return VP_OK;
}
int check_render(unsigned what, const Param* p, long long last_frame)
{
    if (what & CHK_STATE)
    {
        if (!G.have_volume) return fail(VP_E_STATE, "render before init_cuda");
        if (!G.have_env) return fail(VP_E_STATE, "render before init_envmap");
        if (!G.have_sun) return fail(VP_E_STATE, "render before set_sun");
        if (!G.have_cam) return fail(VP_E_STATE, "render before copy_inv_view_matrix");
    }
    if ((what & CHK_IMAGE) && (p->width == 0 || p->height == 0 || p->width > 65535 || p->height > 65535))
        return fail(VP_E_ARG, (what & CHK_IMAGE_NOTE) ? "image %ux%u out of range (sampler.h packs x<<16|y)" : "image %ux%u out of range", p->width, p->height);
    if (what & CHK_MODES)
    {
        if (G.trk && G.env_mis) return fail(VP_E_STATE, "scalar tracking builds exist with passive environment lighting only");
        if (G.trk && G.count) return fail(VP_E_STATE, "work counters are not built for the scalar tracking kernels");
        if (G.rng == VP_RNG_PHILOX7 && (G.trk || G.env_mis))
            return fail(VP_E_STATE, "VP_RNG_PHILOX7 is built for spectral tracking with passive environment lighting only");
        if (G.arith == VP_ARITH_FAST)
        {
            if (G.rng == VP_RNG_SAMPLERH) return fail(VP_E_STATE, "VP_ARITH_FAST is not built for VP_RNG_SAMPLERH (the parity mode is exact by definition)");
            if (G.est == VP_EST_BOUNDED) return fail(VP_E_STATE, "VP_ARITH_FAST is not built for VP_EST_BOUNDED");
            if (G.env_mis) return fail(VP_E_STATE, "VP_ARITH_FAST is built for passive environment lighting only");
            if (G.trk) return fail(VP_E_STATE, "VP_ARITH_FAST is built for spectral tracking only");
            if (G.count) return fail(VP_E_STATE, "work counters are not built for VP_ARITH_FAST");
        }
        if (int rc = subpixel_check(p)) return rc;
    }
    if ((what & CHK_OPACITY) && G.est == VP_EST_DECOMP && last_frame > 10 && !G.S.opacity)
        return fail(VP_E_NOOPACITY, "frames beyond 10 need precompute_opacity (kernel.cu:2183, host.cpp:336-343)");
    return VP_OK;
}
static bool approach_built()
{
    const bool dense_volume = G.marked_fraction > G.dense_fraction;
    return G.use_approach && !G.sub_shift && (G.est == VP_EST_GLOBAL || (G.est == VP_EST_DECOMP && G.use_approach_local && !dense_volume)) && !G.trk && !G.env_mis;
}
static bool approach_possible(const float4* crawl, unsigned n_general) { return approach_built() && crawl && n_general; }
struct LaunchPlan
{
    Target     T;
    bool       lookahead;
    bool       stage_only;
    const StatsDev* stats;
    float4*    layers;
    unsigned integrated_end() const { return PL.n_general + ((PL.n_light && !light_const) ? PL.n_light : 0u); }
    PixelLists PL;
    size_t     per_frame;
    bool       staged;
    bool       light_const;
    bool       approach, approach_thr, appr_aux_needed;
    bool       piped; int slot;
    size_t     max_f;
    bool both() const { return PL.n_light && PL.n_general && !light_const; }
    size_t sized_frames(int f) const { return std::min<size_t>(stage_only ? std::max<size_t>((size_t)f, (size_t)std::max(G.la_max, 1)) : (size_t)f, max_f); }
};
static int prepare_tables(const Param* p, const Shard& sh, int nframes, const PixelLists* lists, LaunchDev& L, LaunchPlan& A)
{
    int rc = VP_OK;
    L.sub_shift = (unsigned)G.sub_shift;
    const Param fine = subpixel_param(p);
    if ((rc = ensure_crawl_table(&fine, &L.crawl))) return rc;
    if ((rc = ensure_pixel_lists(p, L.crawl, sh))) return rc;
    const PixelLists& PL = A.PL = lists ? *lists : PixelLists{G.d_tiles, G.n_general, G.n_light, G.n_miss};
    A.per_frame = (size_t)PL.n_general + PL.n_light + PL.n_miss;
    if (A.per_frame == 0) return VP_OK;
    if ((rc = ensure_sun_clip(&L.sun_clip, &L.clip_ds))) return rc;
    L.count_clips = getenv("VP_DEBUG_COUNT_CLIPS") ? 1u : 0u;
    if ((rc = exit_flights(L))) return rc;
    A.light_const = false;
    if (PL.n_light && (rc = ensure_light_const(p, &A.light_const))) return rc;
    G.last_light_const = A.light_const ? 1 : 0;
    if (G.est == VP_EST_GLOBAL && PL.n_light && !A.light_const)
    {
        if ((rc = ensure_thr_table(p, &L.thr_table))) return rc;
        L.thr_n = G.thr_entries;
    }
    A.approach = A.approach_thr = false;
    if (approach_possible(L.crawl, PL.n_general) && (!G.count || getenv("VP_COUNT_APPROACH")))
    {
        bool identity = true;
        if (G.est == VP_EST_GLOBAL) rc = G.arith == VP_ARITH_FAST ? ensure_fast_identity(p, &identity) : ensure_light_identity(p, &identity);
        if (rc) return rc;
        A.approach = identity || G.arith != VP_ARITH_FAST;
        if (!identity && A.approach)
        {
            if ((rc = ensure_thr_table(p, &L.thr_table))) return rc;
            L.thr_n  = G.thr_entries;
            A.approach_thr = true;
        }
    }
    L.seg_table = nullptr;
    if (A.approach && G.est == VP_EST_DECOMP && G.approach_fshift_max >= 6 && !lists)
    {
        const float4* seg = nullptr;
        if ((rc = ensure_segment_table(p, L.crawl, &seg))) return rc;
        if (nframes >= 64) L.seg_table = seg;
    }
    return VP_OK;
}
static int plan_target(int nframes, const Target* tgt, const PixelLists* lists, LaunchPlan& A)
{
    A.staged = nframes > 1 || A.stage_only || A.stats || A.layers;
    A.T      = tgt ? *tgt : Target{&G.target[0], G.stream};
    A.max_f  = A.staged ? stage_frames_cap(A.per_frame, A.T.rt->stage.bytes) : 1;
    A.appr_aux_needed = A.approach && G.est == VP_EST_DECOMP && A.staged;
    A.slot  = G.pipe_next;
    A.piped = !tgt && !A.stage_only && !lists && !A.stats && !A.layers && nframes > 1 && G.pipeline && !G.count && pipe_target(A.per_frame, nframes, A.appr_aux_needed, &A.T);
    if (A.piped) A.max_f = (size_t)nframes;
    else if (!tgt) G.pipe_fence = true;
    G.last_pipelined = A.piped ? 1 : 0;
    if (!A.appr_aux_needed) return VP_OK;
    const size_t one = A.per_frame * sizeof(uint2);
    return reserve_handover(A.T, one * std::min<size_t>((size_t)nframes, A.max_f), one * A.sized_frames(nframes));
}
static int reserve_launch_stage(LaunchPlan& A, int f, bool* smaller)
{
    *smaller = false;
    const size_t exact = A.per_frame * (size_t)f * sizeof(float4);
// ... 7 lines not shown
}

static int brick_table_form(const LaunchPlan& A, const Param* p, const SceneDev& S)
{
    const bool lds_bounds = G.use_lds_bounds && G.est == VP_EST_DECOMP && G.quant && !G.env_mis && !G.trk &&
                            (size_t)S.bnx * S.bny * S.bnz <= (size_t)VP_LDS_BOUND_ENTRIES;
    const bool ach_lds = p->sigma_t.x == p->sigma_t.y && p->sigma_t.y == p->sigma_t.z && p->albedo.x == p->albedo.y && p->albedo.y == p->albedo.z;
    const bool timed_l  = !G.count && !A.lookahead;
    const bool timed_cb = timed_l && G.rng != VP_RNG_SAMPLERH;
    return !lds_bounds ? 0 : (G.bound_codes_ok && G.d_bound_codes && timed_cb && (ach_lds || G.lds_compact_chromatic)) ? 2
                             : (timed_l && !G.lds_pairs) ? 0 : 1;
}
static bool brick_table_helper(const LaunchPlan& A, int lds_form) { return lds_form == 1 && G.lds_helper && A.PL.n_general && !(A.PL.n_light && !A.light_const) && !A.lookahead; }
struct ClassGrid { bool ldsb; unsigned blocks, cap, wait_iters; };
static ClassGrid class_grid(const LaunchPlan& A, int cls, int lds_form, unsigned total_items)
{
    ClassGrid g;
    g.ldsb = lds_form == 1 && !cls;
    const unsigned bsz  = g.ldsb ? VP_BLOCK_LDS : VP_BLOCK;
    unsigned waves  = (total_items + 63) / 64;
    g.blocks = (waves + (bsz / 64) - 1) / (bsz / 64);
    const bool     both = A.both();
    unsigned       bpc  = G.blocks_per_cu;
    if (both && cls) bpc = G.light_blocks_per_cu ? G.light_blocks_per_cu : (G.est == VP_EST_GLOBAL ? 2u : 6u);
    if (!both && cls) bpc = 8u;
    if (both && !cls) bpc = G.general_blocks_per_cu ? G.general_blocks_per_cu : (G.est == VP_EST_GLOBAL ? 4u : 5u);
    if (A.lookahead && !cls && !both) bpc = std::min(bpc, G.est == VP_EST_GLOBAL ? 6u : 5u);
    g.cap = (unsigned)G.num_cu * (g.ldsb ? 2u : bpc);
    if (g.blocks > g.cap) g.blocks = g.cap;
    g.wait_iters = cls ? (G.light_wait_iters ? G.light_wait_iters : (G.est == VP_EST_GLOBAL ? 128u : 64u)) : G.wait_iters;
    return g;
}
struct AuxBranch
{
    RenderTarget& rt; hipStream_t main; bool forked = false;
    static bool make(hipEvent_t& e) { if (!e && hipEventCreateWithFlags(&e, hipEventDisableTiming) != hipSuccess) { (void)hipGetLastError(); e = nullptr; } return e != nullptr; }
    void fork() { if (!(forked = make(rt.aux_ev[0]) && hipEventRecord(rt.aux_ev[0], main) == hipSuccess)) (void)hipGetLastError(); }
    hipStream_t begin()
    {
        if (!rt.aux_stream && create_internal_stream(&rt.aux_stream) != hipSuccess) { (void)hipGetLastError(); rt.aux_stream = nullptr; }
        if (!make(rt.aux_ev[1]) || !rt.aux_stream || !forked) return nullptr;
        if (hipStreamWaitEvent(rt.aux_stream, rt.aux_ev[0], 0) == hipSuccess) return rt.aux_stream;
        (void)hipGetLastError();
        return nullptr;
    }
    hipError_t join() { return hipEventRecord(rt.aux_ev[1], rt.aux_stream) != hipSuccess || hipStreamWaitEvent(main, rt.aux_ev[1], 0) != hipSuccess ? hipGetLastError() : hipSuccess; }
};
struct Kernels { decltype(&launch_render) render; decltype(&launch_approach) approach; };
struct Launch { const LaunchPlan& A; const SceneDev& S; LaunchDev& L; int f; int lds_form; bool lds_helper; Kernels k; AuxBranch aux; };
static void select_class(const LaunchPlan& A, LaunchDev& L, int cls, int f)
{
    const unsigned nt = cls ? A.PL.n_light : A.PL.n_general;
    L.pixels      = A.PL.pixels + (cls ? A.PL.n_general : 0);
    L.nslots      = nt;
    L.slot_base   = cls ? A.PL.n_general : 0u;
    L.total_items = (unsigned)((size_t)nt * (size_t)f);
    L.queue       = target_queue(A.T.rt) + (cls ? kQueueWords : 0);
    L.chunk_fshift = (!cls && G.chunk_fshift && f % (1 << G.chunk_fshift) == 0) ? G.chunk_fshift : 0u;
    for (unsigned q = 0; q <= VP_NQUEUES; q++) L.q_start[q] = q == VP_NQUEUES ? nt : (unsigned)((unsigned long long)(nt / 64u) * q / VP_NQUEUES) * 64u;
}
static hipError_t launch_general_class(Launch& X, const ClassGrid& g)
{
    const LaunchPlan& A = X.A; LaunchDev& L = X.L; const Target& T = A.T;
    hipError_t le = hipSuccess;
    ClassTimer ct(0, T.stream);
    L.approach = 0;
    G.last_approach = 0;
    G.last_approach_table = 0;
    const bool aux_ok = !A.appr_aux_needed || T.rt->handover.p != nullptr;
    if (A.appr_aux_needed) L.approach_aux = T.rt->handover;
    if (A.approach && aux_ok && L.stage && X.f <= 65535)
    {
        L.approach       = A.approach_thr ? 2u : 1u;
        L.approach_steps = G.approach_steps;
        L.approach_fshift = 0;
        while (L.approach_fshift < G.approach_fshift_max && (2u << L.approach_fshift) <= (unsigned)X.f) L.approach_fshift++;
        X.k.approach(X.S, L, G.est, G.rng, G.quant, T.stream);
        le = hipGetLastError();
        G.last_approach = (int)L.approach;
        G.last_approach_table = (G.est == VP_EST_DECOMP && G.quant && L.seg_table && L.approach_fshift == 6u) ? 1 : 0;
        if (X.lds_helper && X.aux.forked && le == hipSuccess) X.aux.fork();
    }
    if (A.piped && le == hipSuccess)
    {
        if (hipEventRecord(G.pipe_gate[A.slot], T.stream) == hipSuccess) G.pipe_gate_set[A.slot] = true;
        else le = hipGetLastError();
    }
    if (le == hipSuccess)
    {
        X.k.render(X.S, L, G.est, G.rng, G.quant, G.half(), G.count, X.lds_form, G.env_mis, G.trk, (int)g.blocks, T.stream);
        le = hipGetLastError();
    }
    if (X.lds_helper && g.ldsb && le == hipSuccess && X.aux.forked && g.blocks >= g.cap)
        if (hipStream_t hs = X.aux.begin())
        {
            X.k.render(X.S, L, G.est, G.rng, G.quant, G.half(), G.count, 0, G.env_mis, G.trk, G.num_cu, hs);
            le = hipGetLastError();
            if (le == hipSuccess) le = X.aux.join();
        }
    ct.stop();
    return le;
}
static hipError_t launch_light_class(Launch& X, const ClassGrid& g)
{
    const LaunchPlan& A = X.A; const Target& T = A.T;
    hipStream_t ls = nullptr;
    if (!A.light_const && A.both() && G.light_overlap) ls = X.aux.begin();
    ClassTimer ct(1, ls ? ls : T.stream);
    if (A.light_const) launch_miss_fill(X.S, X.L, false, T.stream);
    else launch_render_light(X.S, X.L, G.est, G.rng, G.quant, G.count, (int)g.blocks, ls ? ls : T.stream);
    hipError_t le = hipGetLastError();
    ct.stop();
    if (ls && le == hipSuccess) le = X.aux.join();
    return le;
}
static hipError_t launch_miss_class(Launch& X)
{
    const PixelLists& PL = X.A.PL;
    X.L.pixels      = PL.pixels + PL.n_general + PL.n_light;
    X.L.nslots      = PL.n_miss;
    X.L.slot_base   = PL.n_general + PL.n_light;
    X.L.total_items = 0;
    ClassTimer ct(2, X.A.T.stream);
    launch_miss_fill(X.S, X.L, G.est != VP_EST_GLOBAL, X.A.T.stream);
    const hipError_t le = hipGetLastError();
    ct.stop();
    return le;
}
static int launch_classes(const LaunchPlan& A, const SceneDev& S, LaunchDev& L, const Param* p, int f)
{
    const Target& T = A.T;
    HIPCHK(hipMemsetAsync(target_queue(T.rt), 0, 2 * kQueueWords * sizeof(unsigned), T.stream));
    const int lds_form = brick_table_form(A, p, S);
    G.last_lds_form = lds_form;
    L.bound_codes = lds_form == 2 ? G.d_bound_codes : nullptr;
    L.bound_pal[0] = G.bound_pal[0]; L.bound_pal[1] = G.bound_pal[1];
    hipEvent_t e0 = get_event(), e1 = get_event();
    bool timed = e0 && e1 && hipEventRecord(e0, T.stream) == hipSuccess;
    hipError_t le = hipSuccess;
    Launch X = {A, S, L, f, lds_form, brick_table_helper(A, lds_form),
                G.arith == VP_ARITH_FAST ? Kernels{launch_render_fast, launch_approach_fast} : Kernels{launch_render, launch_approach},
                AuxBranch{*T.rt, T.stream}};
    if ((A.both() && G.light_overlap) || X.lds_helper) X.aux.fork();
    for (int cls = 0; cls < 2 && le == hipSuccess; cls++)
// ... 226 lines not shown
    hipEvent_t end[3] = {G.class_last_end[0], G.class_last_end[1], G.class_last_end[2]};
    for (auto& ev : G.class_events) tot[ev.cls] += span_ms(ev.a, ev.b, end[ev.cls]);
    if (ms) for (int i = 0; i < 3; i++) ms[i] = tot[i];
    if (pixels) { pixels[0] = G.n_general; pixels[1] = G.n_light; pixels[2] = G.n_miss; }
    if (reset)
    {
        for (auto& ev : G.class_events) { put_event(ev.a); if (ev.b != end[ev.cls]) put_event(ev.b); }
        for (int i = 0; i < 3; i++)
            if (end[i] != G.class_last_end[i]) { put_event(G.class_last_end[i]); G.class_last_end[i] = end[i]; }
        G.class_events.clear();
        G.class_ms[0] = G.class_ms[1] = G.class_ms[2] = 0.0;
    }
    return VP_OK;
}
static int prepare_segment_table(const Param* p, const float4* table, const float4** seg)
{
    *seg = nullptr;
    if (G.est == VP_EST_DECOMP && G.approach_fshift_max >= 6 && approach_possible(table, G.n_general)) return ensure_segment_table(p, table, seg);
    return VP_OK;
}
int vp_get_pixel_lists(const Param* p, uint32_t* dst, size_t count, unsigned counts[3])
{
    int rc = vp_prepare(p);
    if (rc) return rc;
    const size_t n = (size_t)G.n_general + G.n_light + G.n_miss;
    if (counts) { counts[0] = G.n_general; counts[1] = G.n_light; counts[2] = G.n_miss; }
    if (dst)
    {
        if (count < n) return fail(VP_E_ARG, "pixel lists hold %zu entries", n);
        if (n) HIPCHK(hipMemcpy(dst, G.d_tiles, n * sizeof(unsigned), hipMemcpyDeviceToHost));
    }
    return VP_OK;
}
int vp_prepare(const Param* p)
{
    int rc = ensure_device();
    if (rc) return rc;
    if (!p) return fail(VP_E_ARG, "vp_prepare: null Param");
    if (!G.have_volume || !G.have_cam) return fail(VP_E_STATE, "vp_prepare needs a volume and a camera");
    if ((rc = check_render(CHK_IMAGE, p))) return rc;
    const Shard sh = shard_of(p);
    if (sh.per_frame == 0)
    {
        G.n_general = G.n_light = G.n_miss = 0; G.tiles_key.clear();
        return VP_OK;
    }
    if ((rc = subpixel_check(p))) return rc;
    const float4 *table = nullptr, *seg = nullptr;
    const unsigned short* sc = nullptr; float ds = 0.0f;
    const float* thr = nullptr;
    const Param fine = subpixel_param(p);
    if ((rc = ensure_crawl_table(&fine, &table))) return rc;
    if ((rc = ensure_pixel_lists(p, table, sh))) return rc;
    if (G.have_sun && (rc = ensure_sun_clip(&sc, &ds))) return rc;
    if (G.est == VP_EST_GLOBAL && G.n_light && (rc = ensure_thr_table(p, &thr))) return rc;
    if ((rc = prepare_segment_table(p, table, &seg))) return rc;
    HIPCHK(hipStreamSynchronize(G.stream));
    return VP_OK;
}
int vp_get_segment_table(const Param* p, float* dst, size_t count, int* cap)
{
    if (cap) *cap = (int)(segment_table_records() / 2u);
    if (!dst) return VP_OK;
    int rc = vp_prepare(p);
    if (rc) return rc;
    const float4 *table = nullptr, *seg = nullptr;
    const Param fine = subpixel_param(p);
    if ((rc = ensure_crawl_table(&fine, &table))) return rc;
    if ((rc = prepare_segment_table(p, table, &seg))) return rc;
    if (!seg) return fail(VP_E_STATE, "no segment table in this configuration (decomposition estimator on a uchar volume, approach walk and table switched on)");
    const size_t need = (size_t)G.n_general * segment_table_records() * 4;
    if (count < need) return fail(VP_E_ARG, "segment table needs %zu floats", need);
    HIPCHK(hipMemcpy(dst, seg, need * sizeof(float), hipMemcpyDeviceToHost));
    return VP_OK;
}
int vp_reserve_frames(const Param* p, int nframes)
{
    int rc = ensure_device();
    if (rc) return rc;
    if (!p || nframes <= 0) return fail(VP_E_ARG, "vp_reserve_frames: bad arguments");
    if ((rc = check_render(CHK_IMAGE, p))) return rc;
    const Shard sh = shard_of(p);
    if (sh.per_frame == 0 || nframes == 1) return VP_OK;
    const Target T      = {&G.target[0], G.stream};
    const size_t f      = std::min<size_t>((size_t)nframes, stage_frames_cap(sh.per_frame, T.rt->stage.bytes));
    const size_t need   = sh.per_frame * f * sizeof(float4);
    const size_t need4  = (G.est == VP_EST_DECOMP && approach_built()) ? sh.per_frame * f * sizeof(uint2) : 0;
    if ((rc = reserve_handover(T, need4, need4))) return rc;
    if (need > T.rt->stage.bytes)
    {
        if (la_quiesce()) return VP_E_NODEVICE;
        HIPCHK(hipStreamSynchronize(G.stream));
        (void)reserve_stage(T, need, need, true);
        if (need > T.rt->stage.bytes) return VP_OK;
    }
    if (G.pipeline && f == (size_t)nframes && pipe_streams()) (void)pipe_reserve(1, sh.per_frame, nframes, need4 > 0);
    return VP_OK;
}
}
```

cuda-volpath_amd/csrc/vp_state.h:

```cpp
#pragma once
#include <hip/hip_runtime.h>

#include <cmath>
#include <cstdarg>
#include <cstdio>
#include <cstdlib>
#include <cstring>
#include <deque>
#include <string>
#include <chrono>
#include <vector>

#include "../../include/volpath.h"
#include "vp_kernels.h"

namespace vph __attribute__((visibility("hidden")))
{
using namespace vp;

inline int bound_radius(int nx, float search_radius)
{
    float cell_size = 2.0f / (float)nx;
    return (int)std::ceil(search_radius / cell_size);
}
// ... 120 lines not shown
    void*       h_opacity_cells = nullptr;
    bool        opacity_lds = true;
    bool        wait_lanes_set = false;
    unsigned    wait_lanes  = VP_WAIT_LANES, wait_iters = VP_WAIT_ITERS, setup_lanes = VP_SETUP_LANES, end_lanes = VP_END_LANES, light_wait_iters = 0;
    unsigned    blocks_per_cu = 8;
    unsigned    chunk_fshift = 0;
    bool        use_lds_bounds = true;
    bool        use_lds_compact = true;
    bool        lds_compact_chromatic = true;
    bool        lds_pairs = false;
    unsigned*   d_bound_codes = nullptr;
    unsigned    bound_pal[2] = {0, 0};
    bool        bound_codes_ok = false;
    bool        lds_helper  = true;
    int         cell_bricks = 0;
    bool        use_crawl_table = true;
    bool        use_empty_table = true;
    bool        use_light   = true;
    bool        use_light_local = true;
    int         debug_only_class = -1;
    DevBuf<unsigned> d_tiles;
    unsigned    n_general   = 0, n_light = 0, n_miss = 0;
    std::vector<unsigned char> tiles_key;
    unsigned*   d_tile_rows = nullptr;
    unsigned*   d_tile_scratch = nullptr;
    std::vector<unsigned char> tiles_shape_key;
    DevBuf<unsigned> d_act, d_act_scratch;
    bool        light_overlap = true;
    unsigned    general_blocks_per_cu = 0, light_blocks_per_cu = 0;
    unsigned char* d_danger = nullptr;
    DevBuf<float4> d_crawl;
    std::vector<unsigned char> crawl_key;
    float       marked_fraction = 0.0f, dense_fraction = 0.40f;
    bool        use_sun_clip = true;
    unsigned short* d_sunclip = nullptr;
    float       sunclip_ds  = 0.0f;
    std::vector<unsigned char> sunclip_key;
    bool        use_light_const = true;
    int         last_approach = 0;
    int         last_approach_table = 0;
    int         last_light_const = 0;
    int         last_lds_form = 0;
    int         arith       = VP_ARITH_EXACT;
    int         last_arith  = VP_ARITH_EXACT;
    int         denoise_form = 0, last_denoise_form = 0;
    int         sub_shift   = subpixel_env_shift();
    DevBuf<unsigned char> d_sub_cls;
    unsigned    la_launched = 0, la_cancelled = 0;
    bool        use_const_rows = true;
    unsigned    last_const_from = 0;
    bool        use_approach_table = true;
    DevBuf<float4> d_seg;
    std::vector<unsigned char> seg_key;
    bool        use_approach_local = true;
    bool        use_approach = true;
    unsigned    approach_fshift_max = 6;
    unsigned    approach_steps = 1u << 20;
    unsigned*   d_light_flag = nullptr;
    bool        bound_mask_valid = false;
    unsigned    h_bound_mask[8] = {};
    bool        use_exit    = true;
    bool        exit_local  = false;
    bool        exit_local_auto = true;
    unsigned    exit_k      = 8;
    unsigned char* d_exit   = nullptr;
    float       light_key[7] = {};
    unsigned long long light_epoch = ~0ull;
    bool        light_const = false;
    float       fast_identity_key[5] = {};
    bool        fast_identity_valid = false, fast_identity = false;
    float*      d_thr       = nullptr;
    float       thr_key[5]  = {};
    bool        thr_valid   = false;
    unsigned    thr_entries = 4096;
    std::deque<std::pair<hipEvent_t, hipEvent_t>> events;
    std::vector<hipEvent_t> event_pool;
    hipEvent_t  last_end    = nullptr;
    double      timed_ms    = 0.0;
    int         timed_n     = 0;
    struct ClassEv { int cls; hipEvent_t a, b; };
    std::deque<ClassEv> class_events;
    double      class_ms[3] = {0.0, 0.0, 0.0};
    hipEvent_t  class_last_end[3] = {nullptr, nullptr, nullptr};
    size_t      max_stage_bytes = (size_t)16 << 30;
    float       inv_model[12] = {1, 0, 0, 0, 0, 1, 0, 0, 0, 0, 1, 0};
    std::string err;
};
State& cur();
#define G vph::cur()
constexpr size_t kMaxPendingEvents = 64;

constexpr size_t kQueueWords = VP_NQUEUES * VP_QUEUE_STRIDE;
constexpr size_t kCounterWords = 76;

int fail(int code, const char* fmt, ...);
[[noreturn]] void die(const char* what);
#define HIPCHK(expr)                                                                            \
    do                                                                                          \
    {                                                                                           \
        hipError_t e_ = (expr);                                                                 \
        if (e_ != hipSuccess)                                                                   \
        {                                                                                       \
            if (e_ == hipErrorOutOfMemory) (void)hipGetLastError();  \
            return fail(e_ == hipErrorOutOfMemory ? VP_E_NOMEM : VP_E_NODEVICE, "%s -> %s", #expr, hipGetErrorString(e_)); \
        }                                                                                       \
    } while (0)

int        ensure_device();
hipError_t create_internal_stream(hipStream_t* st);
int        free_volume();
int        do_init_volume(const void* h_volume, vp_extent ext, int format, const vp_float3* bmin, const vp_float3* bmax);
int        do_envmap(const vp_float4* data, int w, int h);
int        build_env_tables();
hipEvent_t get_event();
inline void put_event(hipEvent_t e) { if (e) G.event_pool.push_back(e); }
struct Shard { unsigned tiles_x, tiles_y, owned; size_t per_frame; };
Shard  shard_of(const Param* p);
size_t stage_frames_cap(size_t per_frame, size_t have_bytes);
int    do_opacity(const float* dir);
int    ensure_crawl_table(const Param* p, const float4** out);
Param  subpixel_param(const Param* p);
int    subpixel_check(const Param* p);
int    ensure_sun_clip(const unsigned short** out, float* ds);
int    ensure_light_const(const Param* p, bool* out);
int    ensure_light_identity(const Param* p, bool* out);
int    ensure_fast_identity(const Param* p, bool* out);
int    ensure_bound_mask();
int    exit_flights(LaunchDev& L);
int    ensure_thr_table(const Param* p, const float** out);
int    ensure_pixel_lists(const Param* p, const float4* table, const Shard& sh);
int    ensure_segment_table(const Param* p, const float4* crawl, const float4** out);
struct Target { RenderTarget* rt; hipStream_t stream; };
struct PixelLists { const unsigned* pixels; unsigned n_general, n_light, n_miss; };
int  do_render(vp_float4* d_out, int first, int nframes, const Param* p, bool stage_only = false, const Target* tgt = nullptr,
               const PixelLists* lists = nullptr, const StatsDev* stats = nullptr, vp_float4* d_trans = nullptr);
enum : unsigned { CHK_STATE = 1, CHK_IMAGE = 2, CHK_IMAGE_NOTE = 4, CHK_MODES = 8, CHK_OPACITY = 16 };
int  check_render(unsigned what, const Param* p, long long last_frame = 0);
void trim_events();
int  pipe_quiesce();
void render_key(const Param* p, std::vector<unsigned char>& key);
bool la_cancel_running();
int  la_quiesce();
int  la_render_slot(int si, vp_float4* d_out, int first, int n, const Param* p, const std::vector<unsigned char>& key);
int  la_limit(int first, int n, size_t per_frame, size_t have_bytes);
int  serve_frame(vp_float4* d_out, int frame, const Param* p);
}
```

cuda-volpath_amd/csrc/vp_tables.cpp:

```cpp
#include "vp_state.h"

namespace vph __attribute__((visibility("hidden")))
{
int do_opacity(const float* dir)
{
    G.epoch++;
    (void)la_quiesce();

    if (!G.have_volume) return fail(VP_E_STATE, "precompute_opacity before init_cuda");
    size_t n = (size_t)G.S.nx * G.S.ny * G.S.nz;
    if (!G.d_opacity) HIPCHK(hipMalloc((void**)&G.d_opacity, n * sizeof(float)));
    SceneDev S = G.S;
    S.linear   = G.linear ? 1 : 0;
    launch_opacity(S, G.quant, G.half(), G.opacity_lds, dir, G.d_opacity, G.stream);
    HIPCHK(hipGetLastError());
    const size_t cbytes = n * 8 * sizeof(float);
    if (G.d_opacity_cells && (G.opacity_cells_on_host != !G.use_opacity_cells))
    {
        if (G.opacity_cells_on_host) HIPCHK(hipHostFree(G.h_opacity_cells)); else HIPCHK(hipFree(G.d_opacity_cells));
        G.d_opacity_cells = nullptr; G.h_opacity_cells = nullptr;
    }
    if (!G.d_opacity_cells)
    {
        G.opacity_cells_on_host = !G.use_opacity_cells;
// ... 252 lines not shown
        G.fast_identity_valid = true;
    }
    *out = G.fast_identity;
    return VP_OK;
}

int ensure_thr_table(const Param* p, const float** out)
{
    *out = nullptr;
    const float key[5] = {p->sigma_t.x, p->sigma_t.y, p->sigma_t.z, p->density, p->g};
    if (!G.thr_valid || !G.d_thr || memcmp(key, G.thr_key, sizeof key) != 0)
    {
        if (la_quiesce()) return VP_E_NODEVICE;
        HIPCHK(hipStreamSynchronize(G.stream));
        if (!G.d_thr) HIPCHK(hipMalloc((void**)&G.d_thr, G.thr_entries * sizeof(float)));
        ParamDev P;
        memcpy(&P, p, sizeof(Param));
        launch_thr_table(P, G.d_thr, G.thr_entries, G.stream);
        HIPCHK(hipGetLastError());
        HIPCHK(hipStreamSynchronize(G.stream));
        memcpy(G.thr_key, key, sizeof key);
        G.thr_valid = true;
    }
    *out = G.d_thr;
    return VP_OK;
}

int ensure_segment_table(const Param* p, const float4* crawl, const float4** out)
{
    *out = nullptr;
    if (!G.use_approach_table || !crawl || !G.quant || G.est != VP_EST_DECOMP || !G.n_general || !G.d_tiles) return VP_OK;
    std::vector<unsigned char> key = G.crawl_key;
    key.insert(key.end(), G.tiles_key.begin(), G.tiles_key.end());
    const size_t need = (size_t)G.n_general * segment_table_records() * sizeof(float4);
    if (key != G.seg_key || !G.d_seg)
    {
        if (la_quiesce()) return VP_E_NODEVICE;
        HIPCHK(hipStreamSynchronize(G.stream));
        if (need > G.d_seg.bytes)
        {
            G.seg_key.clear();
            if (G.d_seg.grow(need) != hipSuccess) return VP_OK;
        }
        SceneDev S = G.S;
        S.linear   = G.linear ? 1 : 0;
        launch_segment_table(S, p->width, p->height, crawl, G.d_tiles, G.n_general, G.d_seg, G.stream);
        HIPCHK(hipGetLastError());
        HIPCHK(hipStreamSynchronize(G.stream));
        G.seg_key = key;
    }
    *out = G.d_seg;
    return VP_OK;
}
int ensure_pixel_lists(const Param* p, const float4* table, const Shard& sh)
{
    const bool light = G.use_light && table && G.trk == VP_TRACK_SPECTRAL && !(G.est != VP_EST_GLOBAL && !G.use_light_local);
    struct K { unsigned w, h, rank, world; int light; };
    std::vector<unsigned char> key(sizeof(K), 0);
    K* k = reinterpret_cast<K*>(key.data());
    k->w = p->width; k->h = p->height; k->rank = G.rank; k->world = G.world; k->light = light ? 1 : 0;
    std::vector<unsigned char> shape_key = key;
    key.push_back((unsigned char)G.sub_shift);
    if (light) key.insert(key.end(), G.crawl_key.begin(), G.crawl_key.end());
    if (key == G.tiles_key && G.d_tiles) return VP_OK;
    if (la_quiesce()) return VP_E_NODEVICE;
    HIPCHK(hipStreamSynchronize(G.stream));
    if ((size_t)sh.owned * 64 > (size_t)0xffffffffu) return fail(VP_E_ARG, "image too large for the 32-bit pixel-list index");
    const unsigned nblocks = pixel_list_blocks(sh.owned);
    if (shape_key != G.tiles_shape_key || !G.d_tile_rows)
    {
        std::vector<unsigned> rows(sh.tiles_y + 1, 0);
        for (unsigned ty = 0; ty < sh.tiles_y; ty++)
        {
            const unsigned first = (G.rank + G.world - tile_row_shift(ty, G.world)) % G.world;
            rows[ty + 1] = rows[ty] + (first < sh.tiles_x ? (sh.tiles_x - first + G.world - 1) / G.world : 0u);
        }
        if (rows[sh.tiles_y] != sh.owned) return fail(VP_E_STATE, "tile enumeration disagrees with the shard (%u vs %u tiles)", rows[sh.tiles_y], sh.owned);
        if (G.d_tile_rows) HIPCHK(hipFree(G.d_tile_rows));
        if (G.d_tile_scratch) HIPCHK(hipFree(G.d_tile_scratch));
        G.d_tile_rows = G.d_tile_scratch = nullptr; G.tiles_shape_key.clear();
        HIPCHK(hipMalloc((void**)&G.d_tile_rows, rows.size() * sizeof(unsigned)));
        HIPCHK(hipMalloc((void**)&G.d_tile_scratch, ((size_t)3 * nblocks + 4) * sizeof(unsigned)));
        HIPCHK(hipMemcpyAsync(G.d_tile_rows, rows.data(), rows.size() * sizeof(unsigned), hipMemcpyHostToDevice, G.stream));
        HIPCHK(hipStreamSynchronize(G.stream));
        G.tiles_shape_key = shape_key;
    }
    if (sh.per_frame * sizeof(unsigned) > G.d_tiles.bytes)
    {
        G.tiles_key.clear();
        HIPCHK(G.d_tiles.grow(sh.per_frame * sizeof(unsigned)));
    }
    unsigned* d_totals = G.d_tile_scratch + (size_t)3 * nblocks;
    const unsigned char* cls = nullptr;
    if (light && G.sub_shift)
    {
        HIPCHK(G.d_sub_cls.grow((size_t)p->width * p->height));
        launch_subpixel_classes(table, p->width, p->height, (unsigned)G.sub_shift, G.d_sub_cls, G.stream);
        HIPCHK(hipGetLastError());
        cls = G.d_sub_cls;
    }
    launch_pixel_lists(p->width, p->height, G.rank, G.world, sh.owned, G.d_tile_rows, light ? table : nullptr, cls, G.d_tile_scratch, d_totals, G.d_tiles, G.stream);
    HIPCHK(hipGetLastError());
    unsigned totals[3] = {0, 0, 0};
    HIPCHK(hipMemcpyAsync(totals, d_totals, sizeof totals, hipMemcpyDeviceToHost, G.stream));
    HIPCHK(hipStreamSynchronize(G.stream));
    if ((size_t)totals[0] + totals[1] + totals[2] != sh.per_frame)
// ... 97 lines not shown
```

cuda-volpath_amd/csrc/vp_test_kernels.h:

```cpp

__global__ void test_hg_k(const float* g, const float* r0, const float* r1, const float* nrm, const float* cosq, float* dir, float* ev, int n)
{
    int i = threadIdx.x + blockIdx.x * blockDim.x;
    if (i >= n) return;
    Frame fr(f3{nrm[3 * i], nrm[3 * i + 1], nrm[3 * i + 2]});
    f3    d = normalize(fr.to_world(hg_sample_local(g[i], r0[i], r1[i])));
    dir[3 * i] = d.x; dir[3 * i + 1] = d.y; dir[3 * i + 2] = d.z;
    ev[i] = hg_eval(g[i], cosq[i]);
}
__global__ void test_math_k(int which, const float* in, float* out, int n)
{
    int i = threadIdx.x + blockIdx.x * blockDim.x;
    if (i >= n) return;
    float x = in[i], s, c, r;
    switch (which)
    {
        case 0: r = logf_(x); break;
        case 1: r = expf_(x); break;
        case 2: sincosf_(x, s, c); r = s; break;
        case 3: sincosf_(x, s, c); r = c; break;
        case 4: r = acosf_(x); break;
        case 5: r = atanf_(x); break;
        case 6: r = pow15f_(x); break;
        case 7: r = rcp_(x); break;
// ... 122 lines not shown
                unsigned long long n_steps = 0;
                through = approach_segment_walk(dist, t_box, t_empty, inv_sigma, rng, sa, sb, n_steps) ? 1u : 0u;
                steps   = (unsigned)n_steps;
            }
        }
        unsigned* o = (ref ? out_ref : out_new) + 5 * (size_t)i;
        o[0] = f2u(dist); o[1] = steps; o[2] = sa; o[3] = sb; o[4] = through;
    }
}

__device__ __forceinline__ bool sun_start_ref_(f3 ro, f3 end, const SceneDev& S, f3& sd_out, float& len_out, float& tn, float& tf)
{
    const f3    dv = end - ro;
    const float d2 = dot(dv, dv);
    const float len = sqrt_(d2);
#ifdef VP_ARITH_FAST
    f3 sd = dv * rsqrt_(d2);
#else
    f3 sd = dv * rcp_(len);
#endif
    bool  hitv = intersect_box(ro, sd, S, tn, tf);
    sd_out = sd; len_out = len;
    return hitv;
}
__global__ void test_sun_start_k(int n, const float* origin, float sun_x, float sun_y, float sun_z, const float* box, unsigned* out_new, unsigned* out_ref)
{
    const f3 sun_dir = f3{sun_x, sun_y, sun_z};
    __shared__ float row[SR_WORDS];
    __shared__ float lbox[6];
    if (threadIdx.x == 0) sun_row_fill(row, sun_dir);
    if (threadIdx.x < 6) lbox[threadIdx.x] = box[threadIdx.x];
    __syncthreads();
    const int i = threadIdx.x + blockIdx.x * blockDim.x;
    if (i >= n) return;
    const f3 ro = f3{origin[3 * (size_t)i], origin[3 * (size_t)i + 1], origin[3 * (size_t)i + 2]};
    {
        f3       sd;
        float    len, tn, tf;
        unsigned taken = 0;
        const bool hit = sun_start(row, ro, lbox, lbox + 3, sd, len, tn, tf, &taken);
        unsigned* o = out_new + 8 * (size_t)i;
        o[0] = f2u(sd.x); o[1] = f2u(sd.y); o[2] = f2u(sd.z); o[3] = f2u(len); o[4] = f2u(tn); o[5] = f2u(tf); o[6] = hit ? 1u : 0u; o[7] = taken;
    }
    {
        SceneDev S = {};
        for (int c = 0; c < 3; c++) { S.bmin[c] = lbox[c]; S.bmax[c] = lbox[3 + c]; }
        f3    sd;
        float len, tn, tf;
        const bool hit = sun_start_ref_(ro, sun_dir * 1e10f, S, sd, len, tn, tf);
        unsigned* o = out_ref + 8 * (size_t)i;
        o[0] = f2u(sd.x); o[1] = f2u(sd.y); o[2] = f2u(sd.z); o[3] = f2u(len); o[4] = f2u(tn); o[5] = f2u(tf); o[6] = hit ? 1u : 0u; o[7] = 0u;
    }
}
```

cuda-volpath_amd/volpath/__init__.py:

```python
import ctypes as C
import os

import numpy as np

_HERE = os.path.dirname(os.path.abspath(__file__))
LIB_PATH = os.environ.get("VOLPATH_LIB", os.path.join(os.path.dirname(_HERE), "libvolpath_hip.so"))

EST_GLOBAL, EST_DECOMP, EST_BOUNDED = 0, 1, 2
RNG_SAMPLERH, RNG_PHILOX, RNG_PHILOX7 = 0, 1, 2
ENV_PASSIVE, ENV_MIS = 0, 1
TRACK_SPECTRAL, TRACK_SCALAR, TRACK_MULTI_CHANNEL = 0, 1, 2
ARITH_EXACT, ARITH_FAST = 0, 1
VOL_U8, VOL_F32, VOL_F16 = 0, 1, 2
ARITH_FAST_REL_L2 = 2e-3
SUBPIXEL_MAX = 8

PART1_SYMBOLS = ["init_cuda", "set_texture_filter_mode", "free_cuda_buffers", "precompute_opacity", "init_envmap",
                 "free_envmap", "set_sun", "copy_inv_view_matrix", "copy_inv_model_matrix", "init_rng", "free_rng",
                 "render_kernel", "scale", "gamma_correct"]
PART2_SYMBOLS = ["vp_last_error", "vp_version", "vp_device_count", "vp_set_device", "vp_set_stream", "vp_get_stream", "vp_synchronize",
                 "vp_set_estimator", "vp_set_rng", "vp_set_envmap_sampling", "vp_get_env_tables", "vp_set_lookahead", "vp_set_tracking", "vp_set_bound_brick", "vp_set_shard", "vp_render_frames", "vp_init_volume", "vp_get_volume_info",
                 "vp_enable_counters", "vp_read_counters", "vp_render_time_ms", "vp_get_bound_table", "vp_get_opacity", "vp_get_pixel_table", "vp_get_null_collision_table", "vp_get_sun_clip_table", "vp_get_exit_table", "vp_set_exit_flights", "vp_render_class_time_ms", "vp_last_approach_mode", "vp_last_approach_table", "vp_last_light_const", "vp_last_lds_form", "vp_set_arithmetic", "vp_last_arithmetic", "vp_set_subpixel", "vp_get_subpixel", "vp_subpixel_offset", "vp_set_pipeline", "vp_last_pipelined", "vp_lookahead_stats", "vp_prepare", "vp_reserve_frames", "vp_get_pixel_lists", "vp_get_segment_table",
                 "vp_render_frames_stats", "vp_render_adaptive", "vp_scale_by_count", "vp_stats_rel_error",
                 "vp_denoise", "vp_set_denoise_form", "vp_last_denoise_form",
                 "vp_render_frames_layers", "vp_composite",
                 "vp_julia_voxelize", "vp_cloud_voxelize", "vp_test_math", "vp_test_rng", "vp_test_sample_density", "vp_test_hg", "vp_test_roots", "vp_test_log_forms", "vp_test_approach_walk", "vp_test_sun_start", "vp_test_launch_census", "vp_test_intersect_box",
                 "vp_test_eval_envmap", "vp_ctx_create", "vp_ctx_destroy", "vp_ctx_set_current", "vp_ctx_get_current", "vp_ctx_device",
                 "vp_accumulate", "vp_tile_owner", "vp_malloc", "vp_free", "vp_memset",
                 "vp_upload", "vp_download"]


class Float3(C.Structure):
    _fields_ = [("x", C.c_float), ("y", C.c_float), ("z", C.c_float)]


class Dim3(C.Structure):
    _fields_ = [("x", C.c_uint32), ("y", C.c_uint32), ("z", C.c_uint32)]


class VolumeInfo(C.Structure):
    _fields_ = [("format", C.c_int), ("nx", C.c_int), ("ny", C.c_int), ("nz", C.c_int), ("cell_bytes", C.c_int),
                ("cells_bytes", C.c_uint64)]


class Extent(C.Structure):
    _fields_ = [("width", C.c_size_t), ("height", C.c_size_t), ("depth", C.c_size_t)]


class Param(C.Structure):
    _fields_ = [("width", C.c_uint32), ("height", C.c_uint32), ("density", C.c_float), ("brightness", C.c_float),
                ("albedo", Float3), ("g", C.c_float), ("sigma_t", Float3)]


class Counters(C.Structure):
    _fields_ = [(n, C.c_uint64) for n in ("samples", "density_lookups", "density_loads", "bound_lookups",
                                          "opacity_lookups", "env_lookups", "scatters", "rng_draws")]

    def as_dict(self):
        return {n: int(getattr(self, n)) for n, _ in self._fields_}


class PixelStats(C.Structure):
    _fields_ = [("sum_y", C.c_double), ("sum_y2", C.c_double), ("n", C.c_uint32), ("flags", C.c_uint32)]


PIXEL_STATS_DTYPE = np.dtype([("sum_y", np.float64), ("sum_y2", np.float64), ("n", np.uint32), ("flags", np.uint32)])
STATS_FROZEN = 1


class Adaptive(C.Structure):
    _fields_ = [("rel_tol", C.c_float), ("floor_y", C.c_float), ("min_frames", C.c_int), ("round_frames", C.c_int)]


class AdaptiveResult(C.Structure):
    _fields_ = [("samples", C.c_uint64), ("rounds", C.c_uint32), ("active_left", C.c_uint32), ("frames_used", C.c_uint32)]

    def as_dict(self):
        return {n: int(getattr(self, n)) for n, _ in self._fields_}

# ... 2 lines not shown
    _fields_ = [("radius", C.c_int), ("patch", C.c_int), ("k", C.c_float)]


DENOISE_MAX_RADIUS, DENOISE_MAX_PATCH = 10, 3


class VolpathError(RuntimeError):
    pass


_lib = None


def lib():
    global _lib
    if _lib is None:
        if not os.path.exists(LIB_PATH):
            raise VolpathError(f"{LIB_PATH} is missing: run `make -C cuda-volpath_amd` (or __graft_entry__.build())")
        L = C.CDLL(LIB_PATH)
        L.vp_last_error.restype = C.c_char_p
        L.vp_version.restype = C.c_char_p
        L.vp_malloc.restype = C.c_void_p
        L.vp_malloc.argtypes = [C.c_size_t]
        L.vp_free.argtypes = [C.c_void_p]
        L.vp_memset.argtypes = [C.c_void_p, C.c_int, C.c_size_t]
        L.vp_upload.argtypes = [C.c_void_p, C.c_void_p, C.c_size_t]
        L.vp_download.argtypes = [C.c_void_p, C.c_void_p, C.c_size_t]
        L.vp_set_stream.argtypes = [C.c_void_p]
        L.vp_get_stream.restype = C.c_void_p
        L.vp_set_rng.argtypes = [C.c_int, C.c_uint32, C.c_uint32]
        L.vp_get_env_tables.argtypes = [C.c_void_p, C.c_void_p, C.POINTER(C.c_float)]
        L.vp_render_frames.argtypes = [C.c_void_p, C.c_int, C.c_int, C.POINTER(Param)]
        L.vp_render_frames_stats.argtypes = [C.c_void_p, C.c_void_p, C.c_int, C.c_int, C.POINTER(Param)]
        L.vp_render_adaptive.argtypes = [C.c_void_p, C.c_void_p, C.c_int, C.c_int, C.POINTER(Param), C.POINTER(Adaptive), C.POINTER(AdaptiveResult)]
        L.vp_scale_by_count.argtypes = [C.c_void_p, C.c_void_p, C.c_void_p, C.c_int, C.c_float]
        L.vp_stats_rel_error.argtypes = [C.c_void_p, C.c_void_p, C.c_int, C.c_float]
        L.vp_denoise.argtypes = [C.c_void_p] * 5 + [C.c_int, C.c_int, C.POINTER(DenoiseParams)]
        L.vp_set_denoise_form.argtypes = [C.c_int]
        L.vp_render_frames_layers.argtypes = [C.c_void_p, C.c_void_p, C.c_int, C.c_int, C.POINTER(Param)]
        L.vp_composite.argtypes = [C.c_void_p] * 4 + [C.POINTER(C.c_float), C.c_int, C.c_float]
        L.vp_read_counters.argtypes = [C.POINTER(Counters), C.c_int]
        L.vp_render_time_ms.argtypes = [C.POINTER(C.c_double), C.POINTER(C.c_int), C.c_int]
        L.vp_get_bound_table.argtypes = [C.c_void_p, C.c_size_t] + [C.POINTER(C.c_int)] * 5
        L.vp_get_opacity.argtypes = [C.c_void_p, C.c_size_t]
        L.vp_get_pixel_table.argtypes = [C.POINTER(Param), C.c_void_p, C.c_size_t]
        L.vp_get_null_collision_table.argtypes = [C.POINTER(Param), C.c_void_p, C.c_size_t]
        L.vp_get_sun_clip_table.argtypes = [C.c_void_p, C.c_size_t, C.POINTER(C.c_float)]
        L.vp_render_class_time_ms.argtypes = [C.POINTER(C.c_double), C.POINTER(C.c_uint32), C.c_int]
        L.vp_prepare.argtypes = [C.POINTER(Param)]
        L.vp_set_subpixel.argtypes = [C.c_int]
        L.vp_subpixel_offset.argtypes = [C.c_uint, C.c_uint, C.c_int, C.c_int, C.POINTER(C.c_int), C.POINTER(C.c_int)]
        L.vp_get_pixel_lists.argtypes = [C.POINTER(Param), C.c_void_p, C.c_size_t, C.POINTER(C.c_uint32)]
        L.vp_get_segment_table.argtypes = [C.POINTER(Param), C.c_void_p, C.c_size_t, C.POINTER(C.c_int)]
        L.vp_julia_voxelize.argtypes = [C.c_int, C.c_void_p]
        L.vp_cloud_voxelize.argtypes = [C.c_int, C.c_uint32, C.c_void_p]
        L.vp_test_math.argtypes = [C.c_int, C.c_void_p, C.c_void_p, C.c_int]
        L.vp_test_roots.argtypes = [C.c_int, C.c_uint32, C.c_uint32, C.POINTER(C.c_uint64), C.POINTER(C.c_uint32)]
        L.vp_test_log_forms.argtypes = [C.c_int, C.c_uint32, C.c_uint32, C.POINTER(C.c_uint64), C.POINTER(C.c_uint32)]
        L.vp_test_approach_walk.argtypes = [C.c_int, C.c_int, C.c_void_p, C.c_void_p, C.c_void_p, C.c_uint32, C.c_void_p, C.c_void_p]
        L.vp_test_sun_start.argtypes = [C.c_int, C.c_void_p, C.c_void_p, C.c_void_p, C.c_void_p, C.c_void_p]
        L.vp_test_launch_census.argtypes = [C.c_int, C.c_int, C.c_void_p, C.c_void_p, C.c_size_t, C.c_int]
        L.vp_test_rng.argtypes = [C.c_int] + [C.c_uint32] * 5 + [C.c_int, C.c_void_p]
        L.vp_test_sample_density.argtypes = [C.c_void_p, C.c_void_p, C.c_int]
        L.vp_test_hg.argtypes = [C.c_void_p] * 7 + [C.c_int]
        L.vp_test_intersect_box.argtypes = [C.c_void_p] * 5 + [C.c_int]
        L.vp_test_eval_envmap.argtypes = [C.c_void_p, C.c_void_p, C.c_int]
        L.vp_ctx_create.restype = C.c_void_p
        L.vp_ctx_create.argtypes = [C.c_int]
        L.vp_ctx_destroy.argtypes = [C.c_void_p]
        L.vp_ctx_set_current.argtypes = [C.c_void_p]
        L.vp_ctx_get_current.restype = C.c_void_p
        L.vp_accumulate.argtypes = [C.c_void_p, C.c_void_p, C.c_size_t]
        L.vp_tile_owner.argtypes = [C.c_uint, C.c_uint, C.c_int]
        L.init_cuda.argtypes = [C.c_void_p, Extent, C.c_bool, C.POINTER(Float3), C.POINTER(Float3)]
        L.init_cuda.restype = None
        L.vp_init_volume.argtypes = [C.c_void_p, Extent, C.c_int, C.POINTER(Float3), C.POINTER(Float3)]
        L.vp_get_volume_info.argtypes = [C.POINTER(VolumeInfo)]
        L.set_texture_filter_mode.argtypes = [C.c_bool]
        L.precompute_opacity.argtypes = [C.POINTER(C.c_float)]
        L.init_envmap.argtypes = [C.c_void_p, C.c_int, C.c_int]
        L.set_sun.argtypes = [C.POINTER(C.c_float), C.POINTER(C.c_float)]
        L.copy_inv_view_matrix.argtypes = [C.POINTER(C.c_float), C.c_size_t]
        L.copy_inv_model_matrix.argtypes = [C.POINTER(C.c_float), C.c_size_t]
        L.init_rng.argtypes = [Dim3, Dim3, C.c_int, C.c_int]
        L.render_kernel.argtypes = [Dim3, Dim3, C.c_void_p, C.c_int, C.POINTER(Param)]
        L.scale.argtypes = [C.c_void_p, C.c_void_p, C.c_int, C.c_float]
        L.gamma_correct.argtypes = [C.c_void_p, C.c_void_p, C.c_int, C.c_float, C.c_float]
        for name in ("set_texture_filter_mode", "free_cuda_buffers", "precompute_opacity", "init_envmap",
                     "free_envmap", "set_sun", "copy_inv_view_matrix", "copy_inv_model_matrix", "init_rng",
                     "free_rng", "render_kernel", "scale", "gamma_correct"):
            getattr(L, name).restype = None
        _lib = L
    return _lib


def _chk(rc):
    if rc != 0:
        raise VolpathError(f"volpath error {rc}: {lib().vp_last_error().decode()}")


def _p(a):
    return a.ctypes.data_as(C.c_void_p)


def device_count():
    return lib().vp_device_count()
# ... 319 lines not shown
    _chk(lib().vp_prepare(C.byref(P)))


def pixel_lists(P):
    cnt = (C.c_uint32 * 3)()
    _chk(lib().vp_get_pixel_lists(C.byref(P), None, 0, cnt))
    n = sum(cnt[:])
    out = np.empty(max(n, 1), np.uint32)
    _chk(lib().vp_get_pixel_lists(C.byref(P), _p(out), n, cnt))
    a, b = cnt[0], cnt[0] + cnt[1]
    return out[:a], out[a:b], out[b:n]


def bound_table(quantized=True):
    bnx, bny, bnz, brick, radius = (C.c_int() for _ in range(5))
    _chk(lib().vp_get_bound_table(None, 0, bnx, bny, bnz, brick, radius))
    out = np.empty((bnz.value, bny.value, bnx.value, 2), np.uint8 if quantized else np.float32)
    _chk(lib().vp_get_bound_table(_p(out), out.nbytes, bnx, bny, bnz, brick, radius))
    return out, brick.value, radius.value


def sun_clip_table(shape):
    out = np.empty(shape, np.uint16)
    step = C.c_float()
    _chk(lib().vp_get_sun_clip_table(_p(out), out.size, C.byref(step)))
    return out, step.value


def set_exit_flights(mode):
    _chk(lib().vp_set_exit_flights(mode))


def exit_table(shape):
    out = np.empty((3,) + tuple(shape), np.uint8)
    _chk(lib().vp_get_exit_table(_p(out), out.size))
    return out


def pixel_table(P):
    out = np.empty((P.height, P.width, 8), np.float32)
    _chk(lib().vp_get_pixel_table(C.byref(P), _p(out), out.size))
    return out


def segment_table(P):
    cap = C.c_int()
    _chk(lib().vp_get_segment_table(C.byref(P), None, 0, C.byref(cap)))
    n = len(pixel_lists(P)[0])
    out = np.empty((n, 2, cap.value, 4), np.float32)
    _chk(lib().vp_get_segment_table(C.byref(P), _p(out), out.size, C.byref(cap)))
    return out[:, 0], out[:, 1], cap.value


def null_collision_table(P, count):
    out = np.empty(count, np.float32)
    _chk(lib().vp_get_null_collision_table(C.byref(P), _p(out), out.size))
    return out


def opacity_table(shape):
    out = np.empty(shape, np.float32)
    _chk(lib().vp_get_opacity(_p(out), out.size))
    return out


def test_math(which, x):
    x = np.ascontiguousarray(x, np.float32)
    out = np.empty_like(x)
    _chk(lib().vp_test_math(which, _p(x), _p(out), x.size))
    return out


def test_roots(which, lo_bits, hi_bits):
    m, f = C.c_uint64(0), C.c_uint32(0)
    _chk(lib().vp_test_roots(which, lo_bits, hi_bits, C.byref(m), C.byref(f)))
    return m.value, (None if m.value == 0 else f.value)


def test_log_forms(which, lo_bits, hi_bits):
    m, f = C.c_uint64(0), C.c_uint32(0)
    _chk(lib().vp_test_log_forms(which, lo_bits, hi_bits, C.byref(m), C.byref(f)))
    return m.value, (None if m.value == 0 else f.value)


def test_approach_walk(kind, params, script, words):
    params = np.ascontiguousarray(params, np.float32).reshape(-1, 4)
    script = np.ascontiguousarray(script, np.uint32).reshape(-1, 4)
    words = np.ascontiguousarray(words, np.uint32).ravel()
    n = params.shape[0]
    if script.shape[0] != n:
        raise ValueError("params and script describe different numbers of cases")
    new, ref = np.zeros((n, 5), np.uint32), np.zeros((n, 5), np.uint32)
    _chk(lib().vp_test_approach_walk(kind, n, _p(params), _p(script), _p(words), words.size, _p(new), _p(ref)))
    return new, ref


def test_sun_start(origins, sun_dir, box):
    origins = np.ascontiguousarray(origins, np.float32).reshape(-1, 3)
    sun_dir = np.ascontiguousarray(sun_dir, np.float32).ravel()
    box = np.ascontiguousarray(box, np.float32).ravel()
    if sun_dir.size != 3 or box.size != 6:
        raise ValueError("sun_dir has three components, box six (bmin, bmax)")
    n = origins.shape[0]
    new, ref = np.zeros((n, 8), np.uint32), np.zeros((n, 8), np.uint32)
    _chk(lib().vp_test_sun_start(n, _p(origins), _p(sun_dir), _p(box), _p(new), _p(ref)))
    return new, ref
# ... 10 lines not shown
        walk, rng = divmod(i, 3)
        return f"g{rng}" if walk == 0 else f"t{rng}" if walk == 2 else f"l{rng}{quant}"
    d = []
    for radix in (2, 2, 2, 3, 2, 2, 3, 2, 2, 3):
        i, r = divmod(i, radix)
        d.append(r)
    half, cancel, light, trk, mis, ach, ldsb, count, quant, rng = d
    return f"{i}{rng}.{quant}{count}{ldsb}{ach}{mis}.{trk}{light}{cancel}{half}"


def launch_census(unit, kind, reset=False):
    n = lib().vp_test_launch_census(unit, kind, None, None, 0, 0)
    if n < 0:
        _chk(n)
    launches, built = np.zeros(n, np.uint32), np.zeros(n, np.uint8)
    _chk(lib().vp_test_launch_census(unit, kind, _p(launches), _p(built), n, int(reset)))
    return {census_name(kind, i): int(launches[i]) for i in np.flatnonzero(built)}


def test_rng(mode, x, y, frame, n, key=(0, 0)):
    out = np.empty(n, np.float32)
    _chk(lib().vp_test_rng(mode, x, y, frame, key[0], key[1], n, _p(out)))
    return out


def test_sample_density(pos):
    pos = np.ascontiguousarray(pos, np.float32)
    out = np.empty(pos.shape[0], np.float32)
    _chk(lib().vp_test_sample_density(_p(pos), _p(out), pos.shape[0]))
    return out


def test_hg(g, r0, r1, normal, cos_query):
    f = lambda a: np.ascontiguousarray(a, np.float32)
    g, r0, r1, normal, cos_query = f(g), f(r0), f(r1), f(normal), f(cos_query)
    n = g.size
    d = np.empty((n, 3), np.float32)
    e = np.empty(n, np.float32)
    _chk(lib().vp_test_hg(_p(g), _p(r0), _p(r1), _p(normal), _p(cos_query), _p(d), _p(e), n))
    return d, e


def test_intersect_box(origin, direction):
    o = np.ascontiguousarray(origin, np.float32)
    d = np.ascontiguousarray(direction, np.float32)
    n = o.shape[0]
    hit = np.empty(n, np.int32)
    tn = np.empty(n, np.float32)
    tf = np.empty(n, np.float32)
    _chk(lib().vp_test_intersect_box(_p(o), _p(d), _p(hit), _p(tn), _p(tf), n))
    return hit.astype(bool), tn, tf


def test_eval_envmap(direction):
    d = np.ascontiguousarray(direction, np.float32)
    out = np.empty_like(d)
    _chk(lib().vp_test_eval_envmap(_p(d), _p(out), d.shape[0]))
    return out


class Context:

    def __init__(self, device=0):
        self.h = lib().vp_ctx_create(device)
        if not self.h:
            raise VolpathError(lib().vp_last_error().decode())
        self._prev = []

    def __enter__(self):
        self._prev.append(lib().vp_ctx_get_current())
        _chk(lib().vp_ctx_set_current(self.h))
        return self

    def __exit__(self, *exc):
        _chk(lib().vp_ctx_set_current(self._prev.pop()))

    def destroy(self):
        if self.h:
            _chk(lib().vp_ctx_destroy(self.h))
            self.h = None


def accumulate(dst_ptr, src_ptr, n_float4):
    _chk(lib().vp_accumulate(dst_ptr, src_ptr, n_float4))


def tile_owner(tx, ty, world):
    return lib().vp_tile_owner(tx, ty, world)


def julia_volume(n):
    out = np.empty((n, n, n), np.uint8)
    _chk(lib().vp_julia_voxelize(n, _p(out)))
    return out


def cloud_volume(n, seed=1):
    out = np.empty((n, n, n), np.float32)
    _chk(lib().vp_cloud_voxelize(n, seed, _p(out)))
    return out


def scale(dst_ptr, src_ptr, n, s):
    lib().scale(dst_ptr, src_ptr, n, s)


# ... 3 lines not shown
```

include/volpath.h:

```cpp
#ifndef VOLPATH_H
#define VOLPATH_H

#include <stddef.h>
#include <stdint.h>
#ifndef __cplusplus
#include <stdbool.h>
#endif

#ifdef __cplusplus
extern "C" {
#endif

typedef struct { float x, y, z; } vp_float3;
typedef struct { float x, y, z, w; } vp_float4;
typedef struct { uint32_t x, y, z; } vp_dim3;
typedef struct { size_t width, height, depth; } vp_extent;

#ifndef VOLPATH_PARAM_DEFINED
#define VOLPATH_PARAM_DEFINED
typedef struct Param
{
    unsigned int width, height;
    float        density, brightness;
    vp_float3    albedo;
// ... 88 lines not shown
typedef struct { uint64_t samples; uint32_t rounds, active_left, frames_used; } vp_adaptive_result;
int vp_render_frames_stats(vp_float4* d_output, vp_pixel_stats* d_stats, int first_frame, int n_frames, const Param* p);
int vp_render_adaptive(vp_float4* d_output, vp_pixel_stats* d_stats, int first_frame, int max_frames, const Param* p,
                       const vp_adaptive* a, vp_adaptive_result* result);
int vp_scale_by_count(vp_float4* dst, const vp_float4* src, const vp_pixel_stats* d_stats, int size, float scale);
int vp_stats_rel_error(float* dst, const vp_pixel_stats* d_stats, int size, float floor_y);

typedef struct { int radius, patch; float k; } vp_denoise_params;
#define VP_DENOISE_MAX_RADIUS 10
#define VP_DENOISE_MAX_PATCH  3
int vp_denoise(vp_float4* dst, const vp_float4* src, const vp_pixel_stats* d_stats,
               const vp_float4* guide, const vp_pixel_stats* d_guide_stats,
               int width, int height, const vp_denoise_params* dp);
int vp_set_denoise_form(int form);
int vp_last_denoise_form(void);

int vp_render_frames_layers(vp_float4* d_fg, vp_float4* d_trans, int first_frame, int n_frames, const Param* p);
int vp_composite(vp_float4* dst, const vp_float4* fg, const vp_float4* trans, const vp_float4* plate, const float plate_rgb[3], int size, float scale);

typedef struct
{
    uint64_t samples;
    uint64_t density_lookups;
    uint64_t density_loads;
    uint64_t bound_lookups;
    uint64_t opacity_lookups;
    uint64_t env_lookups;
    uint64_t scatters;
    uint64_t rng_draws;
} vp_counters;
int vp_enable_counters(int on);
int vp_read_counters(vp_counters* out, int reset);

int vp_render_time_ms(double* total_ms, int* launches, int reset);

int vp_render_class_time_ms(double ms[3], unsigned pixels[3], int reset);

int vp_last_approach_mode(void);
int vp_last_approach_table(void);
int vp_last_light_const(void);
int vp_last_lds_form(void);
int vp_last_arithmetic(void);
int vp_set_pipeline(int on);
int vp_last_pipelined(void);
int vp_lookahead_stats(unsigned* launched, unsigned* cancelled_in_flight);
int vp_prepare(const Param* p);
int vp_reserve_frames(const Param* p, int n_frames);
int vp_get_pixel_lists(const Param* p, uint32_t* dst, size_t count, unsigned counts[3]);

int vp_get_bound_table(void* dst, size_t bytes, int* bnx, int* bny, int* bnz, int* brick, int* radius);
int vp_get_opacity(float* dst, size_t count);
int vp_get_pixel_table(const Param* p, float* dst, size_t count);
int vp_get_segment_table(const Param* p, float* dst, size_t count, int* cap);
int vp_get_sun_clip_table(unsigned short* dst, size_t count, float* step);
int vp_get_exit_table(unsigned char* dst, size_t count);
int vp_set_exit_flights(int mode);
int vp_get_null_collision_table(const Param* p, float* dst, size_t count);

int vp_test_math(int which, const float* in, float* out, int n);
int vp_test_roots(int which, uint32_t lo_bits, uint32_t hi_bits, uint64_t* mismatches, uint32_t* first_bad);
int vp_test_log_forms(int which, uint32_t lo_bits, uint32_t hi_bits, uint64_t* mismatches, uint32_t* first_bad);
int vp_test_approach_walk(int kind, int n, const float* params, const uint32_t* script, const uint32_t* words, uint32_t n_words,
                          uint32_t* out_new, uint32_t* out_ref);
int vp_test_sun_start(int n, const float* origin_xyz, const float* sun_dir, const float* box, uint32_t* out_new, uint32_t* out_ref);
int vp_test_launch_census(int unit, int kind, uint32_t* launches, uint8_t* built, size_t count, int reset);
int vp_test_rng(int mode, uint32_t x, uint32_t y, uint32_t frame, uint32_t k0, uint32_t k1, int n, float* out);
int vp_test_sample_density(const float* pos_xyz, float* out, int n);
int vp_test_hg(const float* g, const float* r0, const float* r1, const float* normal_xyz, const float* cos_query, float* dir_xyz,
               float* eval, int n);
int vp_test_intersect_box(const float* origin_xyz, const float* dir_xyz, int* hit, float* tnear, float* tfar, int n);
int vp_test_eval_envmap(const float* dir_xyz, float* rgb, int n);

int vp_julia_voxelize(int n, unsigned char* host_out);
int vp_cloud_voxelize(int n, uint32_t seed, float* host_out);

void* vp_malloc(size_t bytes);
int   vp_free(void* dptr);
int   vp_memset(void* dptr, int value, size_t bytes);
int   vp_upload(void* dptr, const void* src, size_t bytes);
int   vp_download(void* dst, const void* dptr, size_t bytes);

#ifdef __cplusplus
}
#endif
#endif
```

Baseline: 3722 Msamples/s.

## Precompute per-pixel camera ray direction, box interval and empty skip into a table

Adds a per-pixel-slot table, built once per camera/volume/tile configuration, holding the primary ray direction, box entry/exit distances and the empty-space skip distance. The global-majorant integrator reads 32 bytes per new path instead of computing camera_ray, intersect_box and a crawl-table lookup. It also pads the kernel-argument LDS region to a 16-byte boundary for the sun row. This swaps ALU work for memory traffic and an extra table build whenever the key changes. The table is cached across frames, but it is still recomputed when the scene changes, so it is not reuse of stale results.

```diff
diff --git a/cuda-volpath_amd/csrc/vp_context.cpp b/cuda-volpath_amd/csrc/vp_context.cpp
--- a/cuda-volpath_amd/csrc/vp_context.cpp
+++ b/cuda-volpath_amd/csrc/vp_context.cpp
@@ -89,6 +89,7 @@
     if (knob("VP_NO_APPROACH", 0, 1, v)) G.use_approach = v == 0;
     if (knob("VP_NO_APPROACH_LOCAL", 0, 1, v)) G.use_approach_local = v == 0;
     if (knob("VP_NO_APPROACH_TABLE", 0, 1, v)) G.use_approach_table = v == 0;
+    if (knob("VP_NO_RAY_TABLE", 0, 1, v)) G.use_ray_table = v == 0;
     if (knob("VP_APPROACH_FRAMES_LOG2", 0, 6, v)) G.approach_fshift_max = (unsigned)v;
     if (knob("VP_APPROACH_STEPS", 0, 1 << 30, v)) G.approach_steps = (unsigned)v;
     if (knob("VP_NO_LIGHT", 0, 1, v)) G.use_light = v == 0;
@@ -532,7 +533,7 @@
         for (hipEvent_t e : {D.pipe_done[0], D.pipe_done[1], D.pipe_free[0], D.pipe_free[1], D.pipe_gate[0], D.pipe_gate[1], D.pipe_fence_ev, D.last_end,
                              D.class_last_end[0], D.class_last_end[1], D.class_last_end[2]})
             if (e) (void)hipEventDestroy(e);
-        D.d_crawl.release(); D.d_seg.release(); D.d_sub_cls.release(); D.d_tiles.release(); D.d_act.release(); D.d_act_scratch.release();
+        D.d_crawl.release(); D.d_seg.release(); D.d_ray.release(); D.d_sub_cls.release(); D.d_tiles.release(); D.d_act.release(); D.d_act_scratch.release();
         for (void* q : {(void*)D.d_thr, (void*)D.d_sunclip, (void*)D.d_bound_codes, (void*)D.d_light_flag, (void*)D.d_tile_rows, (void*)D.d_tile_scratch})
             if (q) (void)hipFree(q);
         for (RenderTarget& t : D.target)
@@ -651,7 +652,7 @@
     if (shift == G.sub_shift) return VP_OK;
     if (la_quiesce()) return VP_E_NODEVICE;
     G.sub_shift = shift;
-    G.crawl_key.clear(); G.tiles_key.clear(); G.seg_key.clear();
+    G.crawl_key.clear(); G.tiles_key.clear(); G.seg_key.clear(); G.ray_key.clear();
     return VP_OK;
 }
 int vp_get_subpixel(void) { return 1 << G.sub_shift; }
@@ -920,6 +921,31 @@
     HIPCHK(hipMemcpy(tfar, dtf, b, hipMemcpyDeviceToHost));
     return VP_OK;
 }
+int vp_test_camera_ray(unsigned width, unsigned height, const uint32_t* pixels, float* out, int n)
+{
+    if (n < 0) return fail(VP_E_ARG, "vp_test_camera_ray: negative count %d", n);
+    if (!pixels || !out) return fail(VP_E_ARG, "vp_test_camera_ray: null argument");
+    if (!width || !height || width > 65536u || height > 65536u) return fail(VP_E_ARG, "vp_test_camera_ray: image %ux%u out of range", width, height);
+    for (int i = 0; i < n; i++)
+        if ((pixels[i] & 0xffffu) >= width || (pixels[i] >> 16) >= height)
+            return fail(VP_E_ARG, "vp_test_camera_ray: pixel %d (%u, %u) outside the %ux%u image", i, pixels[i] & 0xffffu, pixels[i] >> 16, width, height);
+    if (!G.have_volume || !G.have_cam) return fail(VP_E_STATE, "vp_test_camera_ray needs a volume (the box) and a camera");
+    int rc = ensure_device();
+    if (rc) return rc;
+    if (n == 0) return VP_OK;
+    DevArrays D;
+    const size_t c = (size_t)n;
+    unsigned* dp = (unsigned*)D.get(c * 4);
+    float*    dd = (float*)D.get(c * 24);
+    if (!dp || !dd) return fail(VP_E_NOMEM, "vp_test_camera_ray: no device memory");
+    HIPCHK(hipMemcpy(dp, pixels, c * 4, hipMemcpyHostToDevice));
+    if (G.arith == VP_ARITH_FAST) launch_test_camera_ray_fast(G.S, width, height, dp, dd, n, G.stream);
+    else launch_test_camera_ray(G.S, width, height, dp, dd, n, G.stream);
+    HIPCHK(hipGetLastError());
+    HIPCHK(hipStreamSynchronize(G.stream));
+    HIPCHK(hipMemcpy(out, dd, c * 24, hipMemcpyDeviceToHost));
+    return VP_OK;
+}
 int vp_test_eval_envmap(const float* dir_xyz, float* rgb, int n)
 {
     if (!G.have_env) return fail(VP_E_STATE, "no environment map");
diff --git a/cuda-volpath_amd/csrc/vp_integrator.h b/cuda-volpath_amd/csrc/vp_integrator.h
--- a/cuda-volpath_amd/csrc/vp_integrator.h
+++ b/cuda-volpath_amd/csrc/vp_integrator.h
@@ -166,6 +166,7 @@
     }
     constexpr unsigned KARG_L_   = ((sizeof(SceneDev) + alignof(LaunchDev) - 1) / alignof(LaunchDev)) * alignof(LaunchDev);
     constexpr unsigned KARG_WDS_ = (KARG_L_ + sizeof(LaunchDev) + 3) / 4;
+    constexpr unsigned KARG_ROW_ = (KARG_WDS_ + 3u) & ~3u;
     constexpr bool LOCAL = EST != EST_GLOBAL;
     constexpr bool TAB   = TRK == 0 && LDSB != 1 && !LIGHT && !MIS;
 #ifdef VP_EXP_BOX_PARALLEL
@@ -173,7 +174,7 @@
 #else
     constexpr bool SUNROW = TAB && EST != EST_BOUNDED;
 #endif
-    __shared__ __attribute__((aligned(16))) unsigned kargs_lds_[KARG_WDS_ + (SUNROW ? SR_WORDS : 0)];
+    __shared__ __attribute__((aligned(16))) unsigned kargs_lds_[KARG_ROW_ + (SUNROW ? SR_WORDS : 0)];
     {
         const unsigned* src = (const unsigned*)__builtin_amdgcn_kernarg_segment_ptr();
         for (unsigned w = threadIdx.x; w < KARG_WDS_; w += (LDSB == 1 ? VP_BLOCK_LDS : VP_BLOCK)) kargs_lds_[w] = src[w];
@@ -182,13 +183,14 @@
     if (TAB && threadIdx.x < VP_COLL_ROWS)
         coll_row_fill(coll_tab_[threadIdx.x], (int)threadIdx.x, L.P.g, L.P.density, max3(f3{L.P.sigma_t[0], L.P.sigma_t[1], L.P.sigma_t[2]}), LOCAL);
     if (SUNROW && threadIdx.x == VP_COLL_ROWS)
-        sun_row_fill(reinterpret_cast<float*>(kargs_lds_ + KARG_WDS_), f3{S.sun_dir[0], S.sun_dir[1], S.sun_dir[2]});
+        sun_row_fill(reinterpret_cast<float*>(kargs_lds_ + KARG_ROW_), f3{S.sun_dir[0], S.sun_dir[1], S.sun_dir[2]});
     __syncthreads();
     auto coll_row = [&](int n) __attribute__((always_inline)) -> const float* {
         return TAB ? coll_tab_[n < 0 ? 0 : (n > VP_COLL_ROWS - 1 ? VP_COLL_ROWS - 1 : n)] : nullptr;
     };
     constexpr bool EARLY = RNG::kShadowSubstream && !MIS && !LIGHT;
     constexpr bool APPR = EST == EST_GLOBAL && TRK == 0 && !LIGHT && !MIS;
+    constexpr bool RAYT = EST == EST_GLOBAL && !LIGHT;
     constexpr bool APPR_L = EST == EST_DECOMP && TRK == 0 && !LIGHT && !MIS;
     constexpr bool EXITC = TRK == 0 && !MIS && !LIGHT && EST != EST_BOUNDED && (QUANT || EST == EST_GLOBAL);
     constexpr bool PARK = !MIS;
@@ -207,7 +209,7 @@
     constexpr bool COLD = LDSB != 1 && !LIGHT;
     constexpr int  CS_  = COLD ? VP_BLOCK : 1;
     constexpr int NCOLD = 14 + (DEFER ? (ACH ? 1 : 3) : 0);
-    static_assert(!COLD || (LOCAL ? VP_LOCAL_MIN_WAVES : VP_GLOBAL_MIN_WAVES) * (NCOLD * VP_BLOCK * 4 + KARG_WDS_ * 4 + VP_COLL_ROWS * CR_WORDS * 4 + (SUNROW ? SR_WORDS * 4 : 0) + (LDSB == 2 ? VP_LDS_BOUND_ENTRIES / 4 : 0)) <= VP_LDS_BYTES_PER_CU,
+    static_assert(!COLD || (LOCAL ? VP_LOCAL_MIN_WAVES : VP_GLOBAL_MIN_WAVES) * (NCOLD * VP_BLOCK * 4 + KARG_ROW_ * 4 + VP_COLL_ROWS * CR_WORDS * 4 + (SUNROW ? SR_WORDS * 4 : 0) + (LDSB == 2 ? VP_LDS_BOUND_ENTRIES / 4 : 0)) <= VP_LDS_BYTES_PER_CU,
                   "cold per-path state: more workgroups per CU than the LDS holds -- lower VP_*_MIN_WAVES for this ARCH");
     __shared__ float cold_[COLD ? NCOLD : 1][CS_];
     float* const cold_p = &cold_[0][COLD ? threadIdx.x : 0];
@@ -298,9 +300,9 @@
             if (SUNROW && stage == 0u)
             {
 #ifdef VP_EXP_FLAT_KARGS
-                const float* const srow = reinterpret_cast<const float*>(kargs_lds_ + KARG_WDS_);
+                const float* const srow = reinterpret_cast<const float*>(kargs_lds_ + KARG_ROW_);
 #else
-                const float* const srow = reinterpret_cast<const float*>(kargs_ + KARG_WDS_ * 4u);
+                const float* const srow = reinterpret_cast<const float*>(kargs_ + KARG_ROW_ * 4u);
 #endif
                 hitv = sun_start(srow, ro, S.bmin, S.bmax, sd, len, tn, tf);
             }
@@ -617,6 +619,8 @@
             vp_pad<VP_PAD_END>();
             bool fresh = false;
             bool trans = false;
+            bool  tabfed = false;
+            float tab_near = 0.0f, tab_far = 0.0f;
             tally(B_BG, st == EV_BG);
             if (st == EV_BG)
             {
@@ -720,6 +724,7 @@
                                     }
                                     return (size_t)px + (size_t)py * P.width;
                                 };
+                                float tab_te = 0.0f;
                                 if (!COUNT && L.sub_shift)
                                 {
                                     unsigned si, sj;
@@ -731,7 +736,18 @@
                                 else
                                 {
                                     rng.init(px, py, (unsigned)frame, L.key0, L.key1);
-                                    camera_ray(S, P.width, P.height, px, py, ro, rd);
+                                    const float4* const ray = RAYT ? L.ray : nullptr;
+                                    if (RAYT && ray)
+                                    {
+                                        const float4 e0 = ray[2 * (size_t)rem], e1 = ray[2 * (size_t)rem + 1];
+                                        ro       = f3{S.cam[3], S.cam[7], S.cam[11]};
+                                        rd       = f3{e0.x, e0.y, e0.z};
+                                        tab_near = e0.w;
+                                        tab_far  = e1.x;
+                                        tab_te   = e1.y;
+                                        tabfed   = true;
+                                    }
+                                    else camera_ray(S, P.width, P.height, px, py, ro, rd);
                                 }
                                 if (TRK == 2)
                                 {
@@ -745,7 +761,8 @@
                                 seg = 0;
                                 if (EXITC) terms = L.exit_start;
                                 if (COUNT) ex_clear = false;
-                                if (!LIGHT) t_empty = L.crawl ? L.crawl[2 * table_index() + 1].x : 0.0f;
+                                if (RAYT && tabfed) t_empty = tab_te;
+                                else if (!LIGHT) t_empty = L.crawl ? L.crawl[2 * table_index() + 1].x : 0.0f;
                                 if (LOCAL) dist = -1.0f;
                                 if (APPR && L.approach)
                                 {
@@ -799,7 +816,9 @@
             if (EST == EST_GLOBAL && st == ST_SETUP)
             {
                 float t_near, tf;
-                bool  hit = intersect_box(ro, rd, S, t_near, tf);
+                bool  hit;
+                if (RAYT && tabfed) { t_near = tab_near; tf = tab_far; hit = tf > t_near && tf >= 1e-3f; }
+                else hit = intersect_box(ro, rd, S, t_near, tf);
                 if (!hit) st = EV_BG;
                 else
                 {
diff --git a/cuda-volpath_amd/csrc/vp_kernels.h b/cuda-volpath_amd/csrc/vp_kernels.h
--- a/cuda-volpath_amd/csrc/vp_kernels.h
+++ b/cuda-volpath_amd/csrc/vp_kernels.h
@@ -97,6 +97,7 @@
     const float4* seg_table;
     unsigned sub_shift;
     unsigned layers;
+    const float4* ray;
 };
 
 [[noreturn]] void kernel_not_built();
@@ -117,6 +118,8 @@
 unsigned segment_table_records(void);
 void launch_segment_table(const SceneDev& S, unsigned width, unsigned height, const float4* crawl, const unsigned* pixels, unsigned nslots, float4* seg,
                           hipStream_t st);
+void launch_ray_table(const SceneDev& S, unsigned width, unsigned height, const float4* crawl, const unsigned* pixels, unsigned nslots, float4* table,
+                      hipStream_t st);
 void launch_thr_table(const ParamDev& P, float* table, unsigned count, hipStream_t st);
 void launch_bound_bytes(const unsigned char* bounds, size_t nbricks, unsigned* mask, hipStream_t st);
 void launch_light_identity(const ParamDev& P, bool local, const unsigned* mask, unsigned* flag, hipStream_t st);
@@ -168,6 +171,8 @@
 void launch_test_hg(const float* g, const float* r0, const float* r1, const float* nrm, const float* cosq, float* dir, float* ev, int n, hipStream_t st);
 void launch_test_box(const SceneDev& S, const float* o, const float* d, int* hit, float* tn, float* tf, int n, hipStream_t st);
 void launch_test_env(const SceneDev& S, const float* d, float* out, int n, hipStream_t st);
+void launch_test_camera_ray(const SceneDev& S, unsigned width, unsigned height, const unsigned* pixels, float* dir, int n, hipStream_t st);
+void launch_test_camera_ray_fast(const SceneDev& S, unsigned width, unsigned height, const unsigned* pixels, float* dir, int n, hipStream_t st);
 void launch_test_math(int which, const float* in, float* out, int n, hipStream_t st);
 void launch_test_roots(int which, unsigned lo, unsigned hi, unsigned long long* mismatches, unsigned* first_bad, hipStream_t st);
 void launch_test_hg_fast(const float* g, const float* r0, const float* r1, const float* nrm, const float* cosq, float* dir, float* ev, int n, hipStream_t st);
diff --git a/cuda-volpath_amd/csrc/vp_kernels.hip b/cuda-volpath_amd/csrc/vp_kernels.hip
--- a/cuda-volpath_amd/csrc/vp_kernels.hip
+++ b/cuda-volpath_amd/csrc/vp_kernels.hip
@@ -639,6 +639,22 @@
         ro      = ro + rd * t_far;
         t_empty -= t_far;
     }
+}
+
+__global__ __launch_bounds__(256) void ray_table_k(SceneDev S, unsigned width, unsigned height, const float4* crawl, const unsigned* pixels, unsigned nslots,
+                                                   float4* table)
+{
+    const unsigned slot = blockIdx.x * blockDim.x + threadIdx.x;
+    if (slot >= nslots) return;
+    const unsigned pix = pixels[slot], px = pix & 0xffffu, py = pix >> 16;
+    if (px >= width || py >= height) { table[2 * (size_t)slot] = table[2 * (size_t)slot + 1] = make_float4(0.0f, 0.0f, 0.0f, 0.0f); return; }
+    f3 ro, rd;
+    camera_ray(S, width, height, px, py, ro, rd);
+    float t_near, tf;
+    (void)intersect_box(ro, rd, S, t_near, tf);
+    const float t_empty = crawl ? crawl[2 * ((size_t)px + (size_t)py * width) + 1].x : 0.0f;
+    table[2 * (size_t)slot]     = make_float4(rd.x, rd.y, rd.z, t_near);
+    table[2 * (size_t)slot + 1] = make_float4(tf, t_empty, 0.0f, 0.0f);
 }
 
 __device__ __forceinline__ size_t pack_index(int nx, int ny, int i, int j, int k, int bricks)
@@ -1093,6 +1109,11 @@
 {
     hipLaunchKernelGGL(approach_segments_k, dim3((nslots + 255u) / 256u), dim3(256), 0, st, S, width, height, crawl, pixels, nslots, seg);
 }
+void launch_ray_table(const SceneDev& S, unsigned width, unsigned height, const float4* crawl, const unsigned* pixels, unsigned nslots, float4* table,
+                      hipStream_t st)
+{
+    hipLaunchKernelGGL(ray_table_k, dim3((nslots + 255u) / 256u), dim3(256), 0, st, S, width, height, crawl, pixels, nslots, table);
+}
 void launch_pixel_lists(unsigned width, unsigned height, unsigned rank, unsigned world, unsigned ntiles, const unsigned* d_row_start,
                         const float4* table, const unsigned char* cls, unsigned* d_block_counts, unsigned* d_totals, unsigned* d_out, hipStream_t st)
 {
@@ -1347,6 +1368,10 @@
 {
     hipLaunchKernelGGL(test_sun_start_k, dim3((n + 255) / 256), dim3(256), 0, st, n, origin, sun_dir[0], sun_dir[1], sun_dir[2], box, out_new, out_ref);
 }
+void launch_test_camera_ray(const SceneDev& S, unsigned width, unsigned height, const unsigned* pixels, float* dir, int n, hipStream_t st)
+{
+    hipLaunchKernelGGL(test_camera_ray_k, dim3((n + 255) / 256), dim3(256), 0, st, S, width, height, pixels, dir, n);
+}
 void launch_test_rng(int mode, unsigned x, unsigned y, unsigned f, unsigned k0, unsigned k1, int n, float* out, hipStream_t st)
 {
     if (mode == RNG_PHILOX) hipLaunchKernelGGL(test_rng_k<RngPhilox>, dim3(1), dim3(64), 0, st, x, y, f, k0, k1, n, out);
diff --git a/cuda-volpath_amd/csrc/vp_kernels_fast.hip b/cuda-volpath_amd/csrc/vp_kernels_fast.hip
--- a/cuda-volpath_amd/csrc/vp_kernels_fast.hip
+++ b/cuda-volpath_amd/csrc/vp_kernels_fast.hip
@@ -50,6 +50,10 @@
 {
     hipLaunchKernelGGL(fast::test_approach_walk_k, dim3((n + 63) / 64), dim3(64), 0, st, kind, n, par, scr, words, out_new, out_ref);
 }
+void launch_test_camera_ray_fast(const SceneDev& S, unsigned width, unsigned height, const unsigned* pixels, float* dir, int n, hipStream_t st)
+{
+    hipLaunchKernelGGL(fast::test_camera_ray_k, dim3((n + 255) / 256), dim3(256), 0, st, S, width, height, pixels, dir, n);
+}
 void launch_test_sun_start_fast(int n, const float* origin, const float* sun_dir, const float* box, unsigned* out_new, unsigned* out_ref, hipStream_t st)
 {
     hipLaunchKernelGGL(fast::test_sun_start_k, dim3((n + 255) / 256), dim3(256), 0, st, n, origin, sun_dir[0], sun_dir[1], sun_dir[2], box, out_new, out_ref);
diff --git a/cuda-volpath_amd/csrc/vp_render.cpp b/cuda-volpath_amd/csrc/vp_render.cpp
--- a/cuda-volpath_amd/csrc/vp_render.cpp
+++ b/cuda-volpath_amd/csrc/vp_render.cpp
@@ -190,6 +190,7 @@
     float4*    layers;
     unsigned integrated_end() const { return PL.n_general + ((PL.n_light && !light_const) ? PL.n_light : 0u); }
     PixelLists PL;
+    const float4* ray;
     size_t     per_frame;
     bool       staged;
     bool       light_const;
@@ -209,6 +210,9 @@
     const PixelLists& PL = A.PL = lists ? *lists : PixelLists{G.d_tiles, G.n_general, G.n_light, G.n_miss};
     A.per_frame = (size_t)PL.n_general + PL.n_light + PL.n_miss;
     if (A.per_frame == 0) return VP_OK;
+    A.ray = nullptr;
+    if (!lists && (rc = ensure_ray_table(p, L.crawl, &A.ray))) return rc;
+    G.last_ray_table = 0;
     if ((rc = ensure_sun_clip(&L.sun_clip, &L.clip_ds))) return rc;
     L.count_clips = getenv("VP_DEBUG_COUNT_CLIPS") ? 1u : 0u;
     if ((rc = exit_flights(L))) return rc;
@@ -322,6 +326,7 @@
 {
     const unsigned nt = cls ? A.PL.n_light : A.PL.n_general;
     L.pixels      = A.PL.pixels + (cls ? A.PL.n_general : 0);
+    L.ray         = cls ? nullptr : A.ray;
     L.nslots      = nt;
     L.slot_base   = cls ? A.PL.n_general : 0u;
     L.total_items = (unsigned)((size_t)nt * (size_t)f);
@@ -360,6 +365,7 @@
     {
         X.k.render(X.S, L, G.est, G.rng, G.quant, G.half(), G.count, X.lds_form, G.env_mis, G.trk, (int)g.blocks, T.stream);
         le = hipGetLastError();
+        G.last_ray_table = L.ray ? 1 : 0;
     }
     if (X.lds_helper && g.ldsb && le == hipSuccess && X.aux.forked && g.blocks >= g.cap)
         if (hipStream_t hs = X.aux.begin())
@@ -692,6 +698,8 @@
     const Param fine = subpixel_param(p);
     if ((rc = ensure_crawl_table(&fine, &table))) return rc;
     if ((rc = ensure_pixel_lists(p, table, sh))) return rc;
+    const float4* ray = nullptr;
+    if ((rc = ensure_ray_table(p, table, &ray))) return rc;
     if (G.have_sun && (rc = ensure_sun_clip(&sc, &ds))) return rc;
     if (G.est == VP_EST_GLOBAL && G.n_light && (rc = ensure_thr_table(p, &thr))) return rc;
     if ((rc = prepare_segment_table(p, table, &seg))) return rc;
@@ -714,6 +722,22 @@
     HIPCHK(hipMemcpy(dst, seg, need * sizeof(float), hipMemcpyDeviceToHost));
     return VP_OK;
 }
+int vp_get_ray_table(const Param* p, float* dst, size_t count)
+{
+    if (!p || !dst) return fail(VP_E_ARG, "vp_get_ray_table: null argument");
+    int rc = vp_prepare(p);
+    if (rc) return rc;
+    const float4 *table = nullptr, *ray = nullptr;
+    const Param fine = subpixel_param(p);
+    if ((rc = ensure_crawl_table(&fine, &table))) return rc;
+    if ((rc = ensure_ray_table(p, table, &ray))) return rc;
+    if (!ray) return fail(VP_E_STATE, "no ray table in this configuration (global-majorant estimator, no sub-pixel factor, general pixels, the table switched on)");
+    const size_t need = (size_t)G.n_general * 8;
+    if (count < need) return fail(VP_E_ARG, "ray table needs %zu floats", need);
+    HIPCHK(hipMemcpy(dst, ray, need * sizeof(float), hipMemcpyDeviceToHost));
+    return VP_OK;
+}
+int vp_last_ray_table(void) { return G.last_ray_table; }
 int vp_reserve_frames(const Param* p, int nframes)
 {
     int rc = ensure_device();
diff --git a/cuda-volpath_amd/csrc/vp_state.h b/cuda-volpath_amd/csrc/vp_state.h
--- a/cuda-volpath_amd/csrc/vp_state.h
+++ b/cuda-volpath_amd/csrc/vp_state.h
@@ -196,6 +196,10 @@
     bool        use_approach_table = true;
     DevBuf<float4> d_seg;
     std::vector<unsigned char> seg_key;
+    bool        use_ray_table = true;
+    DevBuf<float4> d_ray;
+    std::vector<unsigned char> ray_key;
+    int         last_ray_table = 0;
     bool        use_approach_local = true;
     bool        use_approach = true;
     unsigned    approach_fshift_max = 6;
@@ -274,6 +278,7 @@
 int    ensure_thr_table(const Param* p, const float** out);
 int    ensure_pixel_lists(const Param* p, const float4* table, const Shard& sh);
 int    ensure_segment_table(const Param* p, const float4* crawl, const float4** out);
+int    ensure_ray_table(const Param* p, const float4* crawl, const float4** out);
 struct Target { RenderTarget* rt; hipStream_t stream; };
 struct PixelLists { const unsigned* pixels; unsigned n_general, n_light, n_miss; };
 int  do_render(vp_float4* d_out, int first, int nframes, const Param* p, bool stage_only = false, const Target* tgt = nullptr,
diff --git a/cuda-volpath_amd/csrc/vp_tables.cpp b/cuda-volpath_amd/csrc/vp_tables.cpp
--- a/cuda-volpath_amd/csrc/vp_tables.cpp
+++ b/cuda-volpath_amd/csrc/vp_tables.cpp
@@ -328,6 +328,33 @@
     *out = G.d_seg;
     return VP_OK;
 }
+int ensure_ray_table(const Param* p, const float4* crawl, const float4** out)
+{
+    *out = nullptr;
+    if (!G.use_ray_table || G.est != VP_EST_GLOBAL || G.sub_shift || !G.n_general || !G.d_tiles) return VP_OK;
+    struct K { float cam[12], cam_z, bmin[3], bmax[3]; unsigned w, h, rank, world, n_general; int crawl; };
+    std::vector<unsigned char> key(sizeof(K), 0);
+    K* k = reinterpret_cast<K*>(key.data());
+    memcpy(k->cam, G.S.cam, sizeof k->cam); k->cam_z = G.S.cam_z;
+    memcpy(k->bmin, G.S.bmin, sizeof k->bmin); memcpy(k->bmax, G.S.bmax, sizeof k->bmax);
+    k->w = p->width; k->h = p->height; k->rank = G.rank; k->world = G.world; k->n_general = G.n_general; k->crawl = crawl ? 1 : 0;
+    if (crawl) key.insert(key.end(), G.crawl_key.begin(), G.crawl_key.end());
+    key.insert(key.end(), G.tiles_key.begin(), G.tiles_key.end());
+    const size_t need = (size_t)G.n_general * 2 * sizeof(float4);
+    if (key != G.ray_key || !G.d_ray)
+    {
+        if (la_quiesce()) return VP_E_NODEVICE;
+        HIPCHK(hipStreamSynchronize(G.stream));
+        G.ray_key.clear();
+        if (G.d_ray.grow(need) != hipSuccess) return VP_OK;
+        launch_ray_table(G.S, p->width, p->height, crawl, G.d_tiles, G.n_general, G.d_ray, G.stream);
+        HIPCHK(hipGetLastError());
+        HIPCHK(hipStreamSynchronize(G.stream));
+        G.ray_key = key;
+    }
+    *out = G.d_ray;
+    return VP_OK;
+}
 int ensure_pixel_lists(const Param* p, const float4* table, const Shard& sh)
 {
     const bool light = G.use_light && table && G.trk == VP_TRACK_SPECTRAL && !(G.est != VP_EST_GLOBAL && !G.use_light_local);
diff --git a/cuda-volpath_amd/csrc/vp_test_kernels.h b/cuda-volpath_amd/csrc/vp_test_kernels.h
--- a/cuda-volpath_amd/csrc/vp_test_kernels.h
+++ b/cuda-volpath_amd/csrc/vp_test_kernels.h
@@ -198,3 +198,16 @@
         o[0] = f2u(sd.x); o[1] = f2u(sd.y); o[2] = f2u(sd.z); o[3] = f2u(len); o[4] = f2u(tn); o[5] = f2u(tf); o[6] = hit ? 1u : 0u; o[7] = 0u;
     }
 }
+
+__global__ void test_camera_ray_k(SceneDev S, unsigned width, unsigned height, const unsigned* pixels, float* out, int n)
+{
+    const int i = threadIdx.x + blockIdx.x * blockDim.x;
+    if (i >= n) return;
+    const unsigned pix = pixels[i];
+    f3 ro, rd;
+    camera_ray(S, width, height, pix & 0xffffu, pix >> 16, ro, rd);
+    float tn, tf;
+    const bool hit = intersect_box(ro, rd, S, tn, tf);
+    float* o = out + 6 * (size_t)i;
+    o[0] = rd.x; o[1] = rd.y; o[2] = rd.z; o[3] = tn; o[4] = tf; o[5] = hit ? 1.0f : 0.0f;
+}
diff --git a/cuda-volpath_amd/volpath/__init__.py b/cuda-volpath_amd/volpath/__init__.py
--- a/cuda-volpath_amd/volpath/__init__.py
+++ b/cuda-volpath_amd/volpath/__init__.py
@@ -20,11 +20,11 @@
                  "render_kernel", "scale", "gamma_correct"]
 PART2_SYMBOLS = ["vp_last_error", "vp_version", "vp_device_count", "vp_set_device", "vp_set_stream", "vp_get_stream", "vp_synchronize",
                  "vp_set_estimator", "vp_set_rng", "vp_set_envmap_sampling", "vp_get_env_tables", "vp_set_lookahead", "vp_set_tracking", "vp_set_bound_brick", "vp_set_shard", "vp_render_frames", "vp_init_volume", "vp_get_volume_info",
-                 "vp_enable_counters", "vp_read_counters", "vp_render_time_ms", "vp_get_bound_table", "vp_get_opacity", "vp_get_pixel_table", "vp_get_null_collision_table", "vp_get_sun_clip_table", "vp_get_exit_table", "vp_set_exit_flights", "vp_render_class_time_ms", "vp_last_approach_mode", "vp_last_approach_table", "vp_last_light_const", "vp_last_lds_form", "vp_set_arithmetic", "vp_last_arithmetic", "vp_set_subpixel", "vp_get_subpixel", "vp_subpixel_offset", "vp_set_pipeline", "vp_last_pipelined", "vp_lookahead_stats", "vp_prepare", "vp_reserve_frames", "vp_get_pixel_lists", "vp_get_segment_table",
+                 "vp_enable_counters", "vp_read_counters", "vp_render_time_ms", "vp_get_bound_table", "vp_get_opacity", "vp_get_pixel_table", "vp_get_null_collision_table", "vp_get_sun_clip_table", "vp_get_exit_table", "vp_set_exit_flights", "vp_render_class_time_ms", "vp_last_approach_mode", "vp_last_approach_table", "vp_last_light_const", "vp_last_lds_form", "vp_set_arithmetic", "vp_last_arithmetic", "vp_set_subpixel", "vp_get_subpixel", "vp_subpixel_offset", "vp_set_pipeline", "vp_last_pipelined", "vp_lookahead_stats", "vp_prepare", "vp_reserve_frames", "vp_get_pixel_lists", "vp_get_segment_table", "vp_get_ray_table", "vp_last_ray_table",
                  "vp_render_frames_stats", "vp_render_adaptive", "vp_scale_by_count", "vp_stats_rel_error",
                  "vp_denoise", "vp_set_denoise_form", "vp_last_denoise_form",
                  "vp_render_frames_layers", "vp_composite",
-                 "vp_julia_voxelize", "vp_cloud_voxelize", "vp_test_math", "vp_test_rng", "vp_test_sample_density", "vp_test_hg", "vp_test_roots", "vp_test_log_forms", "vp_test_approach_walk", "vp_test_sun_start", "vp_test_launch_census", "vp_test_intersect_box",
+                 "vp_julia_voxelize", "vp_cloud_voxelize", "vp_test_math", "vp_test_rng", "vp_test_sample_density", "vp_test_hg", "vp_test_roots", "vp_test_log_forms", "vp_test_approach_walk", "vp_test_sun_start", "vp_test_launch_census", "vp_test_intersect_box", "vp_test_camera_ray",
                  "vp_test_eval_envmap", "vp_ctx_create", "vp_ctx_destroy", "vp_ctx_set_current", "vp_ctx_get_current", "vp_ctx_device",
                  "vp_accumulate", "vp_tile_owner", "vp_malloc", "vp_free", "vp_memset",
                  "vp_upload", "vp_download"]
@@ -133,6 +133,8 @@
         L.vp_subpixel_offset.argtypes = [C.c_uint, C.c_uint, C.c_int, C.c_int, C.POINTER(C.c_int), C.POINTER(C.c_int)]
         L.vp_get_pixel_lists.argtypes = [C.POINTER(Param), C.c_void_p, C.c_size_t, C.POINTER(C.c_uint32)]
         L.vp_get_segment_table.argtypes = [C.POINTER(Param), C.c_void_p, C.c_size_t, C.POINTER(C.c_int)]
+        L.vp_get_ray_table.argtypes = [C.POINTER(Param), C.c_void_p, C.c_size_t]
+        L.vp_test_camera_ray.argtypes = [C.c_uint, C.c_uint, C.c_void_p, C.c_void_p, C.c_int]
         L.vp_julia_voxelize.argtypes = [C.c_int, C.c_void_p]
         L.vp_cloud_voxelize.argtypes = [C.c_int, C.c_uint32, C.c_void_p]
         L.vp_test_math.argtypes = [C.c_int, C.c_void_p, C.c_void_p, C.c_int]
@@ -558,6 +560,17 @@
     return out[:, 0], out[:, 1], cap.value
 
 
+def ray_table(P):
+    n = len(pixel_lists(P)[0])
+    out = np.empty((max(n, 1), 8), np.float32)
+    _chk(lib().vp_get_ray_table(C.byref(P), _p(out), n * 8))
+    return out[:n]
+
+
+def last_ray_table():
+    return int(lib().vp_last_ray_table())
+
+
 def null_collision_table(P, count):
     out = np.empty(count, np.float32)
     _chk(lib().vp_get_null_collision_table(C.byref(P), _p(out), out.size))
@@ -674,6 +687,13 @@
     return hit.astype(bool), tn, tf
 
 
+def test_camera_ray(width, height, pixels):
+    px = np.ascontiguousarray(pixels, np.uint32)
+    out = np.empty((px.shape[0], 6), np.float32)
+    _chk(lib().vp_test_camera_ray(width, height, _p(px), _p(out), px.shape[0]))
+    return out[:, :3].copy(), out[:, 3].copy(), out[:, 4].copy(), out[:, 5] != 0.0
+
+
 def test_eval_envmap(direction):
     d = np.ascontiguousarray(direction, np.float32)
     out = np.empty_like(d)
diff --git a/include/volpath.h b/include/volpath.h
--- a/include/volpath.h
+++ b/include/volpath.h
@@ -164,6 +164,9 @@
 int vp_get_opacity(float* dst, size_t count);
 int vp_get_pixel_table(const Param* p, float* dst, size_t count);
 int vp_get_segment_table(const Param* p, float* dst, size_t count, int* cap);
+int vp_get_ray_table(const Param* p, float* dst, size_t count);
+int vp_last_ray_table(void);
+int vp_test_camera_ray(unsigned width, unsigned height, const uint32_t* pixels, float* out, int n);
 int vp_get_sun_clip_table(unsigned short* dst, size_t count, float* step);
 int vp_get_exit_table(unsigned char* dst, size_t count);
 int vp_set_exit_flights(int mode);
```

New measurement: 3763 Msamples/s, median of 6. +1.1%, better.
